# yoseph007/PQA2

Hardware: AMD Instinct MI355X
Metric: VMAF frames/sec (vif+adm+motion2 -> SVM), device-resident synthetic YUV pairs (higher is better)
Workload: dtype f32; 1 GPU; 2160p 3840x2160 8-bit, vmaf_4k_v0.6.1, 300 frames/GPU; frames_per_gpu=300, frames_total=300, batch=97, frames_per_launch=75, clips_pipelined=True, parallelism=frame-shard x1, 1-frame motion halo, all-gather of records + of scores

## Files before the change

### include/pqa_vmaf.h

```cpp
#ifndef PQA_VMAF_H
#define PQA_VMAF_H

#include <stddef.h>
#include <stdint.h>

#if defined(__GNUC__)
#define PQA_API __attribute__((visibility("default")))
#else
#define PQA_API
#endif

#ifdef __cplusplus
extern "C" {
#endif

typedef enum pqa_status {
  PQA_OK = 0,
  PQA_EINVAL = -1,
  PQA_EDEVICE = -2,
  PQA_ENOMEM = -3,
  PQA_ECANCELLED = -4,
  PQA_ESTATE = -5
} pqa_status;

// ... 217 lines not shown
PQA_API int pqa_cross_sse_device(pqa_ctx* ctx, const void* ref_luma, int64_t ref_row_pitch, int64_t ref_frame_pitch,
                                 int32_t n_ref, const void* dis_luma, int64_t dis_row_pitch, int64_t dis_frame_pitch,
                                 int32_t n_dis, int32_t k_lo, int32_t k_hi, uint64_t* out);

PQA_API int pqa_cross_sse(pqa_ctx* ctx, const void* const* ref_frames, int64_t ref_row_stride, int32_t n_ref,
                          const void* const* dis_frames, int64_t dis_row_stride, int32_t n_dis, int32_t k_lo, int32_t k_hi,
                          uint64_t* out);

PQA_API int pqa_shift_sse_device(pqa_ctx* ctx, const void* ref_luma, int64_t ref_row_pitch, int64_t ref_frame_pitch,
                                 const void* dis_luma, int64_t dis_row_pitch, int64_t dis_frame_pitch, int32_t n_frames,
                                 int32_t radius, uint64_t* out);

PQA_API int pqa_shift_sse(pqa_ctx* ctx, const void* const* ref_frames, int64_t ref_row_stride, const void* const* dis_frames,
                          int64_t dis_row_stride, int32_t n_frames, int32_t radius, uint64_t* out);

PQA_API int pqa_level_stats_device(pqa_ctx* ctx, const void* ref, int64_t ref_row_pitch, int64_t ref_frame_pitch,
                                   const void* dis, int64_t dis_row_pitch, int64_t dis_frame_pitch, int32_t n_frames,
                                   int32_t plane, uint64_t* out);

PQA_API int pqa_level_stats(pqa_ctx* ctx, const void* const* ref_frames, int64_t ref_row_stride, const void* const* dis_frames,
                            int64_t dis_row_stride, int32_t n_frames, int32_t plane, uint64_t* out);

PQA_API int pqa_level_bins(const pqa_ctx* ctx);

enum { PQA_RESAMPLE_BILINEAR = 0, PQA_RESAMPLE_BICUBIC = 1, PQA_RESAMPLE_LANCZOS3 = 2 };
typedef struct pqa_resample_spec {
  uint32_t struct_size, filter;
  uint32_t src_width, src_height, dst_width, dst_height;
  int64_t x0_q16, y0_q16, w_q16, h_q16;
} pqa_resample_spec;
PQA_API int pqa_resample(pqa_ctx* ctx, const pqa_resample_spec* spec, const void* const* src_frames, int64_t src_row_stride,
                         void* const* dst_frames, int64_t dst_row_stride, int32_t n_frames);
PQA_API int pqa_resample_device(pqa_ctx* ctx, const pqa_resample_spec* spec, const void* src, int64_t src_row_pitch,
                                int64_t src_frame_pitch, void* dst, int64_t dst_row_pitch, int64_t dst_frame_pitch,
                                int32_t n_frames);

typedef struct pqa_unpack_spec {
  uint32_t struct_size, format;
  uint32_t width, height;
} pqa_unpack_spec;
PQA_API int pqa_unpack_device(pqa_ctx* ctx, const pqa_unpack_spec* spec, const void* src, int64_t src_row_pitch,
                              int64_t src_frame_pitch, int32_t n_frames, const pqa_device_clip* dst);
PQA_API int pqa_unpack(pqa_ctx* ctx, const pqa_unpack_spec* spec, const void* const* src_frames, int64_t src_row_stride,
                       int32_t n_frames, void* const* dst_planes, const int64_t dst_strides[3]);

enum { PQA_SITE_COSITED = 0, PQA_SITE_CENTRE = 1 };
enum { PQA_CONVERT_GENERIC = 1 };
typedef struct pqa_convert_spec {
  uint32_t struct_size, flags;
  uint32_t src_bits, dst_bits;
  uint32_t luma_width, luma_height;
  uint8_t src_hshift, src_vshift, dst_hshift, dst_vshift;
  uint8_t src_hsite, src_vsite, dst_hsite, dst_vsite;
} pqa_convert_spec;
PQA_API int pqa_format_convert(pqa_ctx* ctx, const pqa_convert_spec* spec, const void* const* src_frames, int64_t src_row_stride,
                               void* const* dst_frames, int64_t dst_row_stride, int32_t n_frames);
PQA_API int pqa_format_convert_device(pqa_ctx* ctx, const pqa_convert_spec* spec, const void* src, int64_t src_row_pitch,
                                      int64_t src_frame_pitch, void* dst, int64_t dst_row_pitch, int64_t dst_frame_pitch,
                                      int32_t n_frames);

typedef struct pqa_flow_spec {
  uint32_t struct_size;
  uint32_t width, height;
  uint32_t tile;
} pqa_flow_spec;
PQA_API int pqa_flow_moments(pqa_ctx* ctx, const pqa_flow_spec* spec, const void* const* ref_frames, int64_t ref_row_stride,
                             const void* const* dis_frames, int64_t dis_row_stride, int32_t n_frames, int64_t* out);
PQA_API int pqa_flow_moments_device(pqa_ctx* ctx, const pqa_flow_spec* spec, const void* ref, int64_t ref_row_pitch,
                                    int64_t ref_frame_pitch, const void* dis, int64_t dis_row_pitch, int64_t dis_frame_pitch,
                                    int32_t n_frames, int64_t* out);

typedef struct pqa_profile_spec {
  uint32_t struct_size;
  uint32_t width, height;
} pqa_profile_spec;
PQA_API int pqa_line_profiles(pqa_ctx* ctx, const pqa_profile_spec* spec, const void* const* frames, int64_t row_stride,
                              int32_t n_frames, uint64_t* out);
PQA_API int pqa_line_profiles_device(pqa_ctx* ctx, const pqa_profile_spec* spec, const void* planes, int64_t row_pitch,
                                     int64_t frame_pitch, int32_t n_frames, uint64_t* out);

typedef struct pqa_tile_spec {
  uint32_t struct_size;
  uint32_t width, height;
  uint32_t tile;
} pqa_tile_spec;
PQA_API int pqa_tile_moments(pqa_ctx* ctx, const pqa_tile_spec* spec, const void* const* ref_frames, int64_t ref_row_stride,
                             const void* const* dis_frames, int64_t dis_row_stride, int32_t n_frames, uint64_t* out);
PQA_API int pqa_tile_moments_device(pqa_ctx* ctx, const pqa_tile_spec* spec, const void* ref, int64_t ref_row_pitch,
                                    int64_t ref_frame_pitch, const void* dis, int64_t dis_row_pitch, int64_t dis_frame_pitch,
                                    int32_t n_frames, uint64_t* out);

typedef struct pqa_band_spec {
  uint32_t struct_size;
  uint32_t width, height;
  uint32_t levels;
} pqa_band_spec;
PQA_API int pqa_band_moments(pqa_ctx* ctx, const pqa_band_spec* spec, const void* const* ref_frames, int64_t ref_row_stride,
                             const void* const* dis_frames, int64_t dis_row_stride, int32_t n_frames, uint64_t* out);
PQA_API int pqa_band_moments_device(pqa_ctx* ctx, const pqa_band_spec* spec, const void* ref, int64_t ref_row_pitch,
                                    int64_t ref_frame_pitch, const void* dis, int64_t dis_row_pitch, int64_t dis_frame_pitch,
                                    int32_t n_frames, uint64_t* out);
PQA_API int pqa_band_sums(void);

typedef struct pqa_temporal_spec {
  uint32_t struct_size;
  uint32_t width, height;
  uint32_t tile;
} pqa_temporal_spec;
PQA_API int pqa_temporal_moments(pqa_ctx* ctx, const pqa_temporal_spec* spec, const void* const* ref_frames,
                                 int64_t ref_row_stride, const void* const* dis_frames, int64_t dis_row_stride, int32_t n_frames,
                                 uint64_t* out);
PQA_API int pqa_temporal_moments_device(pqa_ctx* ctx, const pqa_temporal_spec* spec, const void* ref, int64_t ref_row_pitch,
                                        int64_t ref_frame_pitch, const void* dis, int64_t dis_row_pitch, int64_t dis_frame_pitch,
                                        int32_t n_frames, uint64_t* out);
PQA_API int pqa_temporal_sums(void);

typedef struct pqa_edge_spec {
  uint32_t struct_size;
  uint32_t width, height;
} pqa_edge_spec;
PQA_API int pqa_edge_profiles(pqa_ctx* ctx, const pqa_edge_spec* spec, const void* const* ref_frames, int64_t ref_row_stride,
                              const void* const* dis_frames, int64_t dis_row_stride, int32_t n_frames, uint64_t* out);
PQA_API int pqa_edge_profiles_device(pqa_ctx* ctx, const pqa_edge_spec* spec, const void* ref, int64_t ref_row_pitch,
                                     int64_t ref_frame_pitch, const void* dis, int64_t dis_row_pitch, int64_t dis_frame_pitch,
                                     int32_t n_frames, uint64_t* out);
PQA_API int pqa_edge_sums(void);

PQA_API int pqa_colour_sums(void);
PQA_API int pqa_colour_moments_device(pqa_ctx* ctx, const pqa_device_clip* ref, const pqa_device_clip* dis, int32_t n_frames,
                                      uint32_t lo, uint32_t hi, uint64_t* out);
PQA_API int pqa_colour_moments(pqa_ctx* ctx, const void* const* ref_frames, const int64_t ref_strides[3],
                               const void* const* dis_frames, const int64_t dis_strides[3], int32_t n_frames, uint32_t lo,
                               uint32_t hi, uint64_t* out);

PQA_API int pqa_colour_apply_device(pqa_ctx* ctx, const int32_t m[12], const pqa_device_clip* src, const pqa_device_clip* dst,
                                    int32_t n_frames);
PQA_API int pqa_colour_apply(pqa_ctx* ctx, const int32_t m[12], const void* const* src_frames, const int64_t src_strides[3],
                             void* const* dst_frames, const int64_t dst_strides[3], int32_t n_frames);

enum { PQA_GRAY_LUMA = 0, PQA_GRAY_BT601_FULL = 1 };
PQA_API int pqa_set_luma_gray(pqa_ctx* ctx, uint32_t mode);

enum { PQA_PROF_KERNELS = 17 };
PQA_API int pqa_profile_enable(pqa_ctx* ctx, int on);
PQA_API int pqa_profile_read(pqa_ctx* ctx, int kernel_id, double* total_ms, uint64_t* launches, uint64_t* frames);
PQA_API const char* pqa_profile_kernel_name(int kernel_id);

PQA_API int pqa_debug_vif_march_table(uint16_t* out, int32_t capacity_halfwords);

PQA_API int pqa_debug_vif_march_shape(uint32_t width, uint32_t height, int32_t* out6);

PQA_API int pqa_debug_vif_strip_shape(pqa_ctx* ctx, uint32_t scale, uint32_t n_frames, int32_t* out4);

PQA_API int pqa_debug_ciede2000(const double* lab_pairs, int32_t n, double* de_out);

enum { PQA_CAMBI_PARAM_INTS = 22 };
PQA_API int pqa_debug_cambi_params(uint32_t w, uint32_t h, uint32_t bit_depth, int32_t* out, int32_t cap);

PQA_API int pqa_debug_cambi_cmap(const void* luma, int64_t row_pitch_bytes, uint32_t w, uint32_t h, uint32_t bit_depth,
                                 float* cmap, int64_t cap, double* score);

PQA_API int pqa_debug_psnr_hvs_dct8x8(const int32_t* in, int32_t* out, int32_t n);

enum { PQA_PSNR_HVS_TABLE_FLOATS = 384 };
PQA_API int pqa_debug_psnr_hvs_tables(float* out, int32_t cap);

PQA_API int pqa_debug_psnr_hvs_plane(const void* ref, const void* dis, int64_t row_pitch_bytes, uint32_t w, uint32_t h,
                                     uint32_t bit_depth, uint32_t plane_kind, float* block_err, double* mse);

PQA_API int pqa_debug_xpsnr_blocks(const void* ref, const void* ref_m1, const void* ref_m2, const void* dis,
                                   int64_t row_pitch_bytes, uint32_t w, uint32_t h, uint32_t bit_depth, int32_t hfr,
                                   uint64_t* out, double* wsse);

PQA_API int pqa_debug_siti_plane(const void* cur, const void* prev, int64_t row_pitch_bytes, uint32_t w, uint32_t h,
                                 uint32_t bit_depth, int32_t full_range, float* gmap, double* si_ti);

PQA_API int pqa_debug_resample_table(uint32_t filter, int32_t n_src, int32_t n_dst, int64_t x0_q16, int64_t ext_q16,
                                     int32_t* first, int16_t* coeff, int32_t cap_taps, int32_t* taps);

PQA_API int pqa_debug_colour(uint32_t bit_depth, uint32_t hshift, uint32_t vshift, uint32_t w, uint32_t h,
                             const void* const ref[3], const void* const dis[3], uint32_t lo, uint32_t hi, uint64_t* sums28,
                             const int32_t* m, void* const applied[3]);

#ifdef __cplusplus
}
#endif
#endif
```

### pqa2_amd/_native.py

```python
from __future__ import annotations

import ctypes as C
import os
import subprocess

_HERE = os.path.dirname(os.path.abspath(__file__))
LIB_PATH = os.environ.get("PQA_LIB_PATH") or os.path.join(_HERE, "csrc", "libpqa_vmaf.so")

PQA_OK, PQA_EINVAL, PQA_EDEVICE, PQA_ENOMEM, PQA_ECANCELLED, PQA_ESTATE = 0, -1, -2, -3, -4, -5
FEAT_VIF, FEAT_ADM, FEAT_MOTION, FEAT_PSNR, FEAT_SSIM = 1, 2, 4, 8, 16
FEAT_VMAF = FEAT_VIF | FEAT_ADM | FEAT_MOTION
FEAT_ALL = FEAT_VMAF | FEAT_PSNR | FEAT_SSIM
FEAT_FLOAT_SSIM, FEAT_MS_SSIM = 32, 64
FEAT_CIEDE = 256
FEAT_CAMBI, FEAT_CAMBI_FULL_REF = 512, 1024
FEAT_PSNR_HVS = 2048
FEAT_XPSNR, FEAT_XPSNR_HFR = 4096, 8192
FEAT_SITI, FEAT_SITI_REF_FULL, FEAT_SITI_DIS_FULL = 16384, 32768, 65536
FEAT_INTEGRITY = 131072
FEAT_KNOWN = (FEAT_ALL | FEAT_FLOAT_SSIM | FEAT_MS_SSIM | FEAT_CIEDE | FEAT_CAMBI | FEAT_CAMBI_FULL_REF | FEAT_PSNR_HVS
              | FEAT_XPSNR | FEAT_XPSNR_HFR | FEAT_SITI | FEAT_SITI_REF_FULL | FEAT_SITI_DIS_FULL
              | FEAT_INTEGRITY)
VIF_BORDER_FLOAT, VIF_BORDER_INTEGER = 0, 1
FIXED_VIF, FIXED_MOTION, FIXED_ADM, FIXED_ALL = 1, 2, 4, 7
REC_VIF_NUM, REC_VIF_DEN, REC_ADM_NUM, REC_ADM_DEN, REC_MOTION, REC_SSIM, REC_SSE = 0, 4, 8, 12, 16, 17, 20
RECORD_DOUBLES = 24
EXT_FLOAT_SSIM, EXT_FLOAT_SSIM_LCS, EXT_MS_SSIM, EXT_MS_SSIM_L, EXT_MS_SSIM_C, EXT_MS_SSIM_S, EXT_RESERVED = 0, 1, 4, 5, 10, 15, 20
EXT_CIEDE2000, EXT_CIEDE_MEAN_DE = 20, 21
EXT_CAMBI, EXT_CAMBI_SOURCE = 22, 23
CAMBI_PARAM_INTS = 22
EXT_DOUBLES = 24
EXT2_PSNR_HVS_Y, EXT2_PSNR_HVS_CB, EXT2_PSNR_HVS_CR, EXT2_PSNR_HVS, EXT2_PSNR_HVS_MSE, EXT2_RESERVED = 0, 1, 2, 3, 4, 7
EXT2_DOUBLES = 8
EXT3_XPSNR_Y, EXT3_XPSNR_U, EXT3_XPSNR_V, EXT3_WSSE, EXT3_RESERVED = 0, 1, 2, 3, 6
EXT3_DOUBLES = 8
EXT4_SI, EXT4_TI, EXT4_SI_SOURCE, EXT4_TI_SOURCE, EXT4_RESERVED = 0, 1, 2, 3, 4
EXT4_DOUBLES = 8
EXT5_SAD_PREV, EXT5_BLACK_COUNT, EXT5_RESERVED = 0, 3, 4
EXT5_DOUBLES = 8
EXT_BLOCKS = (
    ("ext", EXT_DOUBLES, FEAT_FLOAT_SSIM | FEAT_MS_SSIM | FEAT_CIEDE | FEAT_CAMBI),
    ("ext2", EXT2_DOUBLES, FEAT_PSNR_HVS),
    ("ext3", EXT3_DOUBLES, FEAT_XPSNR),
    ("ext4", EXT4_DOUBLES, FEAT_SITI),
    ("ext5", EXT5_DOUBLES, FEAT_INTEGRITY),
)
PSNR_HVS_TABLE_FLOATS = 384
PROF_KERNELS = 17
GRAY_LUMA, GRAY_BT601_FULL = 0, 1

EXPORTS = [
    "pqa_version", "pqa_record_doubles", "pqa_ext_doubles", "pqa_ext2_doubles", "pqa_ext3_doubles", "pqa_ext4_doubles", "pqa_ext5_doubles", "pqa_config_init", "pqa_create", "pqa_destroy", "pqa_set_stream",
    "pqa_submit", "pqa_submit_fd", "pqa_submit_fd_run", "pqa_submit_device", "pqa_submit_surfaces", "pqa_submit_packed", "pqa_set_motion_halo", "pqa_set_ref_history", "pqa_set_dis_history", "pqa_set_dis_history_planes", "pqa_set_black_threshold", "pqa_frame_sad", "pqa_frame_sad_device", "pqa_flush", "pqa_collect", "pqa_collect_ext", "pqa_collect_ext2", "pqa_collect_ext3", "pqa_collect_ext4", "pqa_collect_ext5", "pqa_sync",
    "pqa_cancel", "pqa_reset", "pqa_last_error", "pqa_luma_stats_device", "pqa_luma_stats", "pqa_cross_sse_device", "pqa_cross_sse", "pqa_shift_sse_device", "pqa_shift_sse", "pqa_level_stats_device", "pqa_level_stats", "pqa_level_bins", "pqa_resample", "pqa_resample_device", "pqa_unpack", "pqa_unpack_device", "pqa_format_convert", "pqa_format_convert_device", "pqa_flow_moments", "pqa_flow_moments_device", "pqa_line_profiles", "pqa_line_profiles_device", "pqa_tile_moments", "pqa_tile_moments_device", "pqa_band_moments", "pqa_band_moments_device", "pqa_band_sums", "pqa_temporal_moments", "pqa_temporal_moments_device", "pqa_temporal_sums", "pqa_edge_profiles", "pqa_edge_profiles_device", "pqa_edge_sums", "pqa_colour_sums", "pqa_colour_moments", "pqa_colour_moments_device", "pqa_colour_apply", "pqa_colour_apply_device", "pqa_set_luma_gray",
    "pqa_profile_enable",
    "pqa_profile_read", "pqa_profile_kernel_name", "pqa_debug_vif_march_table", "pqa_debug_vif_march_shape", "pqa_debug_vif_strip_shape",
    "pqa_debug_ciede2000", "pqa_debug_cambi_params", "pqa_debug_cambi_cmap", "pqa_debug_psnr_hvs_dct8x8",
    "pqa_debug_psnr_hvs_tables", "pqa_debug_psnr_hvs_plane", "pqa_debug_xpsnr_blocks", "pqa_debug_siti_plane",
    "pqa_debug_resample_table", "pqa_debug_colour",
]


class PqaConfig(C.Structure):
    _fields_ = [
        ("struct_size", C.c_uint32), ("device", C.c_int32), ("width", C.c_uint32), ("height", C.c_uint32),
        ("bit_depth", C.c_uint32), ("n_planes", C.c_uint32), ("chroma_hshift", C.c_uint32),
        ("chroma_vshift", C.c_uint32), ("features", C.c_uint32), ("max_batch", C.c_uint32),
        ("result_capacity", C.c_uint32), ("n_subsample", C.c_uint32),
        ("vif_enhn_gain_limit", C.c_double), ("adm_enhn_gain_limit", C.c_double),
        ("vif_border", C.c_uint32), ("fixed_point", C.c_uint32),
    ]


class PqaDeviceClip(C.Structure):
    _fields_ = [("plane", C.c_void_p * 3), ("row_pitch", C.c_int64 * 3), ("frame_pitch", C.c_int64 * 3)]


SURFACE_NV12, SURFACE_P01X = 1, 2
SURFACE_PLANAR, SURFACE_UYVY, SURFACE_YUYV, SURFACE_V210 = 0, 3, 4, 5
PACKED_FORMATS = {"uyvy422": SURFACE_UYVY, "yuyv422": SURFACE_YUYV, "v210": SURFACE_V210}
PACKED_BIT_DEPTH = {SURFACE_UYVY: 8, SURFACE_YUYV: 8, SURFACE_V210: 10}


class PqaSurfaceClip(C.Structure):
    _fields_ = [("struct_size", C.c_uint32), ("format", C.c_uint32), ("luma", C.c_void_p), ("chroma", C.c_void_p),
                ("luma_row_pitch", C.c_int64), ("luma_frame_pitch", C.c_int64),
                ("chroma_row_pitch", C.c_int64), ("chroma_frame_pitch", C.c_int64)]


class PqaHostClip(C.Structure):
    _fields_ = [("struct_size", C.c_uint32), ("format", C.c_uint32), ("frames", C.POINTER(C.c_void_p)), ("strides", C.c_int64 * 3)]


class PqaUnpackSpec(C.Structure):
    _fields_ = [("struct_size", C.c_uint32), ("format", C.c_uint32), ("width", C.c_uint32), ("height", C.c_uint32)]


SITE_COSITED, SITE_CENTRE = 0, 1
CONVERT_GENERIC = 1
CONVERT_BIT_DEPTHS = (8, 10, 12)


class PqaConvertSpec(C.Structure):
    _fields_ = [("struct_size", C.c_uint32), ("flags", C.c_uint32), ("src_bits", C.c_uint32), ("dst_bits", C.c_uint32),
                ("luma_width", C.c_uint32), ("luma_height", C.c_uint32),
                ("src_hshift", C.c_uint8), ("src_vshift", C.c_uint8), ("dst_hshift", C.c_uint8), ("dst_vshift", C.c_uint8),
                ("src_hsite", C.c_uint8), ("src_vsite", C.c_uint8), ("dst_hsite", C.c_uint8), ("dst_vsite", C.c_uint8)]


RESAMPLE_BILINEAR, RESAMPLE_BICUBIC, RESAMPLE_LANCZOS3 = 0, 1, 2
RESAMPLE_FILTERS = {"bilinear": RESAMPLE_BILINEAR, "bicubic": RESAMPLE_BICUBIC, "lanczos": RESAMPLE_LANCZOS3}
RESAMPLE_MAX_TAPS = 32


class PqaResampleSpec(C.Structure):
    _fields_ = [("struct_size", C.c_uint32), ("filter", C.c_uint32), ("src_width", C.c_uint32), ("src_height", C.c_uint32),
                ("dst_width", C.c_uint32), ("dst_height", C.c_uint32), ("x0_q16", C.c_int64), ("y0_q16", C.c_int64),
                ("w_q16", C.c_int64), ("h_q16", C.c_int64)]


FLOW_TILES = (8, 16, 32, 64)
COLOUR_SUMS = 28
COLOUR_Q = 14
COLOUR_MAX_GAIN, COLOUR_MAX_OFFSET = 1 << 16, 1 << 28


class PqaFlowSpec(C.Structure):
    _fields_ = [("struct_size", C.c_uint32), ("width", C.c_uint32), ("height", C.c_uint32), ("tile", C.c_uint32)]


class PqaProfileSpec(C.Structure):
    _fields_ = [("struct_size", C.c_uint32), ("width", C.c_uint32), ("height", C.c_uint32)]


PROFILE_STRIPE, PROFILE_BAND = 1024, 64


class PqaTileSpec(C.Structure):
    _fields_ = [("struct_size", C.c_uint32), ("width", C.c_uint32), ("height", C.c_uint32), ("tile", C.c_uint32)]


TILE_SUMS, TILE_CHUNK = 6, 8


class PqaBandSpec(C.Structure):
    _fields_ = [("struct_size", C.c_uint32), ("width", C.c_uint32), ("height", C.c_uint32), ("levels", C.c_uint32)]


BAND_SUMS, BAND_CHUNK = 3, 8


class PqaTemporalSpec(C.Structure):
    _fields_ = [("struct_size", C.c_uint32), ("width", C.c_uint32), ("height", C.c_uint32), ("tile", C.c_uint32)]


TEMPORAL_SUMS, TEMPORAL_CHUNK = 7, 8
TEMPORAL_SIGNED = (0, 1, 4, 5)


class PqaEdgeSpec(C.Structure):
    _fields_ = [("struct_size", C.c_uint32), ("width", C.c_uint32), ("height", C.c_uint32)]


EDGE_STRIPE, EDGE_BAND = 1024, 64
EDGE_SUMS, EDGE_CHUNK = 3, 8


class PqaError(RuntimeError):
    def __init__(self, code: int, msg: str):
        super().__init__(f"pqa error {code}: {msg}")
        self.code = code


class PqaCancelled(PqaError):
    pass


def build(force: bool = False) -> str:
    script = os.path.join(_HERE, "csrc", "build.sh")
    if force:
        for f in os.listdir(os.path.join(_HERE, "csrc")):
            if f.endswith(".o"):
                os.remove(os.path.join(_HERE, "csrc", f))
    r = subprocess.run(["bash", script], capture_output=True, text=True)
    if r.returncode != 0:
        raise RuntimeError(f"hipcc build failed:\n{r.stdout}\n{r.stderr}")
    return LIB_PATH


_lib = None


def load():
    global _lib
    if _lib is not None:
        return _lib
    if not os.path.exists(LIB_PATH):
        raise ImportError(
            f"{LIB_PATH} is missing: the MI355X HIP extension is not built (run `python -c 'import "
            f"__graft_entry__ as g; g.build()'` or pqa2_amd/csrc/build.sh).  There is no CPU fallback.")
    try:
        import torch
    except Exception:
        pass
    lib = C.CDLL(LIB_PATH)
    missing = [s for s in EXPORTS if not hasattr(lib, s)]
    if missing:
        raise ImportError(f"{LIB_PATH} lacks symbols {missing}")
    vp, i32, i64, dbl = C.c_void_p, C.c_int32, C.c_int64, C.c_double
    lib.pqa_version.restype = C.c_char_p
    lib.pqa_record_doubles.restype = C.c_int
    lib.pqa_config_init.argtypes = [C.POINTER(PqaConfig), C.c_uint32, C.c_uint32]
    lib.pqa_config_init.restype = None
    lib.pqa_create.argtypes = [C.POINTER(PqaConfig), C.POINTER(vp)]
    lib.pqa_destroy.argtypes = [vp]
    lib.pqa_destroy.restype = None
    lib.pqa_set_stream.argtypes = [vp, vp]
    lib.pqa_submit.argtypes = [vp, i64, C.POINTER(vp * 3), C.POINTER(i64 * 3), C.POINTER(vp * 3), C.POINTER(i64 * 3)]
    lib.pqa_submit_fd.argtypes = [vp, i64, C.c_int, C.POINTER(i64 * 3), C.c_int, C.POINTER(i64 * 3)]
    lib.pqa_submit_fd_run.argtypes = [vp, i64, i32, C.c_int, C.POINTER(i64 * 3), i64, C.c_int, C.POINTER(i64 * 3), i64]
    lib.pqa_submit_device.argtypes = [vp, i64, i32, C.POINTER(PqaDeviceClip), C.POINTER(PqaDeviceClip), vp, i64]
    lib.pqa_submit_surfaces.argtypes = [vp, i64, i32, C.POINTER(PqaSurfaceClip), C.POINTER(PqaSurfaceClip),
                                        C.POINTER(PqaSurfaceClip)]
    lib.pqa_submit_packed.argtypes = [vp, i64, i32, C.POINTER(PqaHostClip), C.POINTER(PqaHostClip)]
    lib.pqa_set_motion_halo.argtypes = [vp, vp, i64]
    lib.pqa_flush.argtypes = [vp]
    lib.pqa_collect.argtypes = [vp, i64, i32, vp]
    lib.pqa_collect_ext.argtypes = [vp, i64, i32, vp, vp]
    lib.pqa_ext_doubles.restype = C.c_int
    lib.pqa_collect_ext2.argtypes = [vp, i64, i32, vp, vp, vp]
    lib.pqa_ext2_doubles.restype = C.c_int
    lib.pqa_collect_ext3.argtypes = [vp, i64, i32, vp, vp, vp, vp]
    lib.pqa_ext3_doubles.restype = C.c_int
    lib.pqa_set_ref_history.argtypes = [vp, vp, i32, i64]
    lib.pqa_collect_ext4.argtypes = [vp, i64, i32, vp, vp, vp, vp, vp]
    lib.pqa_ext4_doubles.restype = C.c_int
    lib.pqa_set_dis_history.argtypes = [vp, vp, i64]
    lib.pqa_collect_ext5.argtypes = [vp, i64, i32, vp, vp, vp, vp, vp, vp]
    lib.pqa_ext5_doubles.restype = C.c_int
    lib.pqa_set_dis_history_planes.argtypes = [vp, C.POINTER(vp * 3), C.POINTER(i64 * 3)]
    lib.pqa_set_black_threshold.argtypes = [vp, C.c_uint32]
    lib.pqa_frame_sad.argtypes = [vp, C.POINTER(vp * 3), C.POINTER(i64 * 3), C.POINTER(vp), C.POINTER(i64 * 3), i32, vp]
    lib.pqa_frame_sad_device.argtypes = [vp, C.POINTER(vp * 3), C.POINTER(i64 * 3), C.POINTER(PqaDeviceClip), i32, vp]
    lib.pqa_sync.argtypes = [vp]
    lib.pqa_cancel.argtypes = [vp]
    lib.pqa_luma_stats_device.argtypes = [vp, vp, i64, i64, i32, C.c_uint32, vp]
    lib.pqa_luma_stats.argtypes = [vp, C.POINTER(vp), i64, i32, C.c_uint32, vp]
    lib.pqa_cross_sse_device.argtypes = [vp, vp, i64, i64, i32, vp, i64, i64, i32, i32, i32, vp]
    lib.pqa_cross_sse.argtypes = [vp, C.POINTER(vp), i64, i32, C.POINTER(vp), i64, i32, i32, i32, vp]
    lib.pqa_shift_sse_device.argtypes = [vp, vp, i64, i64, vp, i64, i64, i32, i32, vp]
    lib.pqa_shift_sse.argtypes = [vp, C.POINTER(vp), i64, C.POINTER(vp), i64, i32, i32, vp]
    lib.pqa_level_stats_device.argtypes = [vp, vp, i64, i64, vp, i64, i64, i32, i32, vp]
    lib.pqa_level_stats.argtypes = [vp, C.POINTER(vp), i64, C.POINTER(vp), i64, i32, i32, vp]
    lib.pqa_level_bins.argtypes = [vp]
    lib.pqa_resample.argtypes = [vp, C.POINTER(PqaResampleSpec), C.POINTER(vp), i64, C.POINTER(vp), i64, i32]
    lib.pqa_resample_device.argtypes = [vp, C.POINTER(PqaResampleSpec), vp, i64, i64, vp, i64, i64, i32]
    lib.pqa_unpack_device.argtypes = [vp, C.POINTER(PqaUnpackSpec), vp, i64, i64, i32, C.POINTER(PqaDeviceClip)]
    lib.pqa_format_convert.argtypes = [vp, C.POINTER(PqaConvertSpec), C.POINTER(vp), i64, C.POINTER(vp), i64, i32]
    lib.pqa_format_convert_device.argtypes = [vp, C.POINTER(PqaConvertSpec), vp, i64, i64, vp, i64, i64, i32]
    lib.pqa_unpack.argtypes = [vp, C.POINTER(PqaUnpackSpec), C.POINTER(vp), i64, i32, C.POINTER(vp), C.POINTER(i64 * 3)]
    lib.pqa_flow_moments.argtypes = [vp, C.POINTER(PqaFlowSpec), C.POINTER(vp), i64, C.POINTER(vp), i64, i32, vp]
    lib.pqa_flow_moments_device.argtypes = [vp, C.POINTER(PqaFlowSpec), vp, i64, i64, vp, i64, i64, i32, vp]
    lib.pqa_line_profiles.argtypes = [vp, C.POINTER(PqaProfileSpec), C.POINTER(vp), i64, i32, vp]
    lib.pqa_line_profiles_device.argtypes = [vp, C.POINTER(PqaProfileSpec), vp, i64, i64, i32, vp]
    lib.pqa_tile_moments.argtypes = [vp, C.POINTER(PqaTileSpec), C.POINTER(vp), i64, C.POINTER(vp), i64, i32, vp]
    lib.pqa_tile_moments_device.argtypes = [vp, C.POINTER(PqaTileSpec), vp, i64, i64, vp, i64, i64, i32, vp]
    lib.pqa_band_moments.argtypes = [vp, C.POINTER(PqaBandSpec), C.POINTER(vp), i64, C.POINTER(vp), i64, i32, vp]
    lib.pqa_band_moments_device.argtypes = [vp, C.POINTER(PqaBandSpec), vp, i64, i64, vp, i64, i64, i32, vp]
    lib.pqa_temporal_moments.argtypes = [vp, C.POINTER(PqaTemporalSpec), C.POINTER(vp), i64, C.POINTER(vp), i64, i32, vp]
    lib.pqa_temporal_moments_device.argtypes = [vp, C.POINTER(PqaTemporalSpec), vp, i64, i64, vp, i64, i64, i32, vp]
    lib.pqa_temporal_sums.argtypes = []
    lib.pqa_temporal_sums.restype = C.c_int
    lib.pqa_edge_profiles.argtypes = [vp, C.POINTER(PqaEdgeSpec), C.POINTER(vp), i64, C.POINTER(vp), i64, i32, vp]
    lib.pqa_edge_profiles_device.argtypes = [vp, C.POINTER(PqaEdgeSpec), vp, i64, i64, vp, i64, i64, i32, vp]
    lib.pqa_edge_sums.argtypes = []
    lib.pqa_edge_sums.restype = C.c_int
    lib.pqa_band_sums.argtypes = []
    lib.pqa_band_sums.restype = C.c_int
    lib.pqa_colour_sums.argtypes = []
    lib.pqa_colour_sums.restype = C.c_int
    lib.pqa_colour_moments_device.argtypes = [vp, C.POINTER(PqaDeviceClip), C.POINTER(PqaDeviceClip), i32, C.c_uint32, C.c_uint32, vp]
    lib.pqa_colour_moments.argtypes = [vp, C.POINTER(vp), C.POINTER(i64 * 3), C.POINTER(vp), C.POINTER(i64 * 3), i32, C.c_uint32, C.c_uint32, vp]
    lib.pqa_colour_apply_device.argtypes = [vp, C.POINTER(i32 * 12), C.POINTER(PqaDeviceClip), C.POINTER(PqaDeviceClip), i32]
    lib.pqa_colour_apply.argtypes = [vp, C.POINTER(i32 * 12), C.POINTER(vp), C.POINTER(i64 * 3), C.POINTER(vp), C.POINTER(i64 * 3), i32]
    lib.pqa_debug_colour.argtypes = [C.c_uint32, C.c_uint32, C.c_uint32, C.c_uint32, C.c_uint32, C.POINTER(vp * 3), C.POINTER(vp * 3),
                                     C.c_uint32, C.c_uint32, vp, C.POINTER(i32 * 12), C.POINTER(vp * 3)]
    lib.pqa_debug_resample_table.argtypes = [C.c_uint32, i32, i32, i64, i64, vp, vp, i32, C.POINTER(i32)]
    lib.pqa_set_luma_gray.argtypes = [vp, C.c_uint32]
    lib.pqa_reset.argtypes = [vp]
    lib.pqa_last_error.argtypes = [vp]
    lib.pqa_last_error.restype = C.c_char_p
    lib.pqa_profile_enable.argtypes = [vp, C.c_int]
    lib.pqa_profile_read.argtypes = [vp, C.c_int, C.POINTER(dbl), C.POINTER(C.c_uint64), C.POINTER(C.c_uint64)]
    lib.pqa_debug_vif_march_table.argtypes = [vp, i32]
    lib.pqa_debug_vif_march_shape.argtypes = [C.c_uint32, C.c_uint32, C.POINTER(i32 * 6)]
    lib.pqa_debug_vif_strip_shape.argtypes = [vp, C.c_uint32, C.c_uint32, C.POINTER(i32 * 4)]
    lib.pqa_debug_ciede2000.argtypes = [vp, i32, vp]
    lib.pqa_debug_cambi_params.argtypes = [C.c_uint32, C.c_uint32, C.c_uint32, vp, i32]
    lib.pqa_debug_cambi_cmap.argtypes = [vp, C.c_int64, C.c_uint32, C.c_uint32, C.c_uint32, vp, C.c_int64, vp]
    lib.pqa_debug_psnr_hvs_dct8x8.argtypes = [vp, vp, i32]
    lib.pqa_debug_psnr_hvs_tables.argtypes = [vp, i32]
    lib.pqa_debug_psnr_hvs_plane.argtypes = [vp, vp, C.c_int64, C.c_uint32, C.c_uint32, C.c_uint32, C.c_uint32, vp, vp]
    lib.pqa_debug_xpsnr_blocks.argtypes = [vp, vp, vp, vp, C.c_int64, C.c_uint32, C.c_uint32, C.c_uint32, i32, vp, vp]
    lib.pqa_debug_siti_plane.argtypes = [vp, vp, C.c_int64, C.c_uint32, C.c_uint32, C.c_uint32, i32, vp, vp]
    lib.pqa_profile_kernel_name.argtypes = [C.c_int]
    lib.pqa_profile_kernel_name.restype = C.c_char_p
    assert lib.pqa_record_doubles() == RECORD_DOUBLES
    assert lib.pqa_ext_doubles() == EXT_DOUBLES
    assert lib.pqa_ext2_doubles() == EXT2_DOUBLES
    assert lib.pqa_ext3_doubles() == EXT3_DOUBLES
    assert lib.pqa_ext4_doubles() == EXT4_DOUBLES
    assert lib.pqa_ext5_doubles() == EXT5_DOUBLES
    assert lib.pqa_colour_sums() == COLOUR_SUMS
    _lib = lib
    return lib
```

### pqa2_amd/csrc/adm.hip

```cpp
#include "kernels.h"
#include "pqa_device.h"

namespace pqa {
namespace {

struct AdmArgs {
  const void* ref;
  const void* dis;
  int64_t row_pitch_r, frame_pitch_r, row_pitch_d, frame_pitch_d;
  int w, h, ow, oh, tiles_x, n_tiles;
  float inv_scale, gain_limit, rf_hv, rf_d;
  float k_hv, k_d;
  int left, top, right, bottom;
  float* ll_ref;
  float* ll_dis;
  int64_t ll_row_pitch_r, ll_frame_pitch_r, ll_row_pitch_d, ll_frame_pitch_d;
  double* partials;
};

constexpr int TW = kAdmTileW, TH = kAdmTileH, GW = TW + 2, GH = TH + 2, NRP = GH / 2;
constexpr int VC = 2 * GW + 2, VP = 128;
static_assert(VC <= 128 && VC <= VP && GH % 2 == 0 && GW <= 64, "one column per lane, rows in pairs");
constexpr int SROWS = GH / 2;
constexpr int NIN = 2 * SROWS + 2;
// ... 98 lines not shown
    const int lcyA = 2 * rp, cyA = cy0 - 1 + lcyA, cyB = cyA + 1;
    f2 s[4][4];
#pragma unroll
    for (int q = 0; q < 4; ++q) {
      if (LLONLY && (q & 1)) continue;
      const f4* p = reinterpret_cast<const f4*>(&V[q][rp][2 * lcxs]);
      const f4 v01 = p[0], v23 = p[1];
      s[q][0] = f2{v01.x, v01.y}; s[q][1] = f2{v01.z, v01.w};
      s[q][2] = f2{v23.x, v23.y}; s[q][3] = f2{v23.z, v23.w};
    }
#define PQA_DWT(c0, c1, c2, c3, t)                                                                        \
  __builtin_elementwise_fma(splat(c3), t[3],                                                              \
                            __builtin_elementwise_fma(splat(c2), t[2], __builtin_elementwise_fma(splat(c1), t[1], splat(c0) * t[0])))
    const f2 ra = PQA_DWT(lo0, lo1, lo2, lo3, s[0]);
    const f2 da = PQA_DWT(lo0, lo1, lo2, lo3, s[2]);
    const bool vA = col_valid && cyA >= 0 && cyA < a.oh, vB = col_valid && cyB >= 0 && cyB < a.oh;
    const bool iA = col_inner && lcyA >= 1 && cyA < a.oh;
    const bool iB = col_inner && lcyA + 1 <= TH && cyB >= 0 && cyB < a.oh;
    if (a.ll_ref) {
      float* lr = a.ll_ref + (int64_t)fr * a.ll_frame_pitch_r;
      float* ld = a.ll_dis + (int64_t)fr * a.ll_frame_pitch_d;
      if (iA) {
        lr[(unsigned)cyA * (unsigned)a.ll_row_pitch_r + (unsigned)cx] = ra.x;
        ld[(unsigned)cyA * (unsigned)a.ll_row_pitch_d + (unsigned)cx] = da.x;
      }
      if (iB) {
        lr[(unsigned)cyB * (unsigned)a.ll_row_pitch_r + (unsigned)cx] = ra.y;
        ld[(unsigned)cyB * (unsigned)a.ll_row_pitch_d + (unsigned)cx] = da.y;
      }
    }
    if (LLONLY) continue;
    const f2 ov = PQA_DWT(hi0, hi1, hi2, hi3, s[0]);
    const f2 oh = PQA_DWT(lo0, lo1, lo2, lo3, s[1]);
    const f2 od = PQA_DWT(hi0, hi1, hi2, hi3, s[1]);
    const f2 tv = PQA_DWT(hi0, hi1, hi2, hi3, s[2]);
    const f2 th = PQA_DWT(lo0, lo1, lo2, lo3, s[3]);
    const f2 td = PQA_DWT(hi0, hi1, hi2, hi3, s[3]);
#undef PQA_DWT
    const f2 ot_dp = __builtin_elementwise_fma(ov, tv, oh * th);
    const f2 o_mag_sq = __builtin_elementwise_fma(ov, ov, oh * oh), t_mag_sq = __builtin_elementwise_fma(tv, tv, th * th);
    const f2 lhs = ot_dp * ot_dp, rhs = splat(cos_1deg_sq) * o_mag_sq * t_mag_sq;
    const bool angA = (ot_dp.x >= 0.0f) && (lhs.x >= rhs.x), angB = (ot_dp.y >= 0.0f) && (lhs.y >= rhs.y);
    const f2 z2 = splat(0.0f);
    const f2 m2 = f2{angA ? a.gain_limit : 1.0f, angB ? a.gain_limit : 1.0f};
    const f2 rh = med3_2(z2, th, oh * m2), rv = med3_2(z2, tv, ov * m2), rd = med3_2(z2, td, od * m2);
    const f2 ah = th - rh, av = tv - rv, ad = td - rd;
    const float gA = fmaf(a.k_d, fabsf(ad.x), a.k_hv * (fabsf(ah.x) + fabsf(av.x)));
    const float gB = fmaf(a.k_d, fabsf(ad.y), a.k_hv * (fabsf(ah.y) + fabsf(av.y)));
    const bool wA = iA && col_win && cyA >= a.top && cyA < a.bottom;
    const bool wB = iB && col_win && cyB >= a.top && cyB < a.bottom;
    const f2 mw = f2{wA ? 1.0f : 0.0f, wB ? 1.0f : 0.0f};
    mwin[k] = mw;
    xs[k][0] = rh * splat(a.rf_hv);
    xs[k][1] = rv * splat(a.rf_hv);
    xs[k][2] = rd * splat(a.rf_d);
    const f2 qh = mw * (oh * oh), qv = mw * (ov * ov), qd = mw * (od * od);
    den_h = f2{fmaf(qh.x, fabsf(oh.x), den_h.x), fmaf(qh.y, fabsf(oh.y), den_h.y)};
    den_v = f2{fmaf(qv.x, fabsf(ov.x), den_v.x), fmaf(qv.y, fabsf(ov.y), den_v.y)};
    den_d = f2{fmaf(qd.x, fabsf(od.x), den_d.x), fmaf(qd.y, fabsf(od.y), den_d.y)};
    if (have) {
      G[lcyA][lcx] = vA ? gA : 0.0f;
      G[lcyA + 1][lcx] = vB ? gB : 0.0f;
    }
  }
  if (LLONLY) {
    if (tid < 6) a.partials[((int64_t)fr * a.n_tiles + tile) * 6 + tid] = 0.0;
    return;
  }
  __syncthreads();

  f2 num_h = f2{0.0f, 0.0f}, num_v = num_h, num_d = num_h;
  {
    const int lx0 = min(max(mirror1(cx - 1, a.ow) - (cx0 - 1), 0), GW - 1);
    const int lx2 = min(max(mirror1(cx + 1, a.ow) - (cx0 - 1), 0), GW - 1);
#pragma unroll
    for (int k = 0; k < NROUND; ++k) {
      const int rp = wave + 4 * k;
      const int lcyA = 2 * rp, cyA = cy0 - 1 + lcyA;
      int ly[4] = {mirror1(cyA - 1, a.oh) - (cy0 - 1), lcyA, lcyA + 1, mirror1(cyA + 2, a.oh) - (cy0 - 1)};
      ly[0] = min(max(ly[0], 0), GH - 1);
      ly[3] = min(max(ly[3], 0), GH - 1);
      float rs[4], c[2];
#pragma unroll
      for (int j = 0; j < 4; ++j) {
        const float m = G[ly[j]][lcxs];
        rs[j] = G[ly[j]][lx0] + m + G[ly[j]][lx2];
        if (j == 1) c[0] = m;
        if (j == 2) c[1] = m;
      }
      const float downA = (cyA + 1 < a.oh) ? rs[2] : rs[1];
      const float upB = (cyA >= 0) ? rs[1] : rs[3];
      const f2 thr = f2{(rs[0] + rs[1] + downA) + c[0], (upB + rs[2] + rs[3]) + c[1]};
      const f2 mw = mwin[k];
#pragma unroll
      for (int t = 0; t < 3; ++t) {
        f2 x = f2{fmaxf(fabsf(xs[k][t].x) - thr.x, 0.0f), fmaxf(fabsf(xs[k][t].y) - thr.y, 0.0f)};
        const f2 x3 = (mw * x) * (x * x);
        if (t == 0) num_h += x3;
        if (t == 1) num_v += x3;
        if (t == 2) num_d += x3;
      }
    }
  }
  const float rf3_hv = a.rf_hv * a.rf_hv * a.rf_hv, rf3_d = a.rf_d * a.rf_d * a.rf_d;
  const float part[6] = {num_h.x + num_h.y, num_v.x + num_v.y, num_d.x + num_d.y,
                         rf3_hv * (den_h.x + den_h.y), rf3_hv * (den_v.x + den_v.y), rf3_d * (den_d.x + den_d.y)};
  double v[6];
  block_sum_f32<6>(part, v, red);
  if (tid == 0) {
    double* out = a.partials + ((int64_t)fr * a.n_tiles + tile) * 6;
#pragma unroll
    for (int i = 0; i < 6; ++i) out[i] = v[i];
  }
}

template <typename T>
__global__ __launch_bounds__(kBlock, 4) void adm_scale_kernel(const AdmArgs a) {
  __shared__ f2 V[4][NRP][VP];
  __shared__ float G[GH][GP];
  __shared__ double red[24];
  const int tile = xcd_remap(blockIdx.x, a.n_tiles);
  const int tx = tile % a.tiles_x, ty = tile / a.tiles_x;
  const int fr = blockIdx.y;
  const int cx0 = tx * TW, cy0 = ty * TH;
  const bool outside = !(cx0 < a.right && cx0 + TW > a.left && cy0 < a.bottom && cy0 + TH > a.top);
  if (outside) {
    if (!a.ll_ref) {
      if (threadIdx.x < 6) a.partials[((int64_t)fr * a.n_tiles + tile) * 6 + threadIdx.x] = 0.0;
      return;
    }
    adm_tile<T, true>(a, V, G, red, tile, tx, ty, fr);
  } else {
    adm_tile<T, false>(a, V, G, red, tile, tx, ty, fr);
  }
}

static float dwt_quant_step(int lambda, int theta) {
  static const double g[3] = {1.501, 1.0, 0.534};
  static const double amp[4][3] = {{0.62171, 0.67234, 0.72709},
                                   {0.34537, 0.41317, 0.49428},
                                   {0.18004, 0.22727, 0.28688},
                                   {0.091401, 0.11792, 0.15214}};
  const float r = (float)(3.0 * 1080 * M_PI / 180.0);
  const float temp = (float)log10(pow(2.0, lambda + 1) * 0.401 * g[theta] / (double)r);
  return (float)(2.0 * 0.495 * pow(10.0, 0.466 * (double)temp * (double)temp) / amp[lambda][theta]);
}

}

float adm_dwt_quant_step(int lambda, int theta) { return dwt_quant_step(lambda, theta); }

hipError_t launch_adm_scale(hipStream_t stream, int scale, Elem elem, PlaneRun ref, PlaneRun dis, int n_frames,
                            int w, int h, float inv_scale, float gain_limit, MutPlaneRun ll_ref,
                            MutPlaneRun ll_dis, double* partials, int mode, int* n_partials) {
  if (n_partials) *n_partials = adm_tiles_x((w + 1) / 2) * adm_tiles_y((h + 1) / 2);
  if (n_frames <= 0) return hipSuccess;
  if (mode != ADM_TILED) {
    hipError_t err = hipSuccess;
    if (launch_adm_march(stream, scale, elem, ref, dis, n_frames, w, h, inv_scale, gain_limit, ll_ref, ll_dis, partials,
                         n_partials, &err))
      return err;
  }
  AdmArgs a{};
  a.ref = ref.base; a.dis = dis.base;
  a.row_pitch_r = ref.row_pitch; a.frame_pitch_r = ref.frame_pitch;
  a.row_pitch_d = dis.row_pitch; a.frame_pitch_d = dis.frame_pitch;
  a.w = w; a.h = h;
  a.ow = (w + 1) / 2; a.oh = (h + 1) / 2;
  a.tiles_x = adm_tiles_x(a.ow);
  a.n_tiles = a.tiles_x * adm_tiles_y(a.oh);
  a.inv_scale = inv_scale; a.gain_limit = gain_limit;
  a.rf_hv = 1.0f / dwt_quant_step(scale, 1);
  a.rf_d = 1.0f / dwt_quant_step(scale, 2);
  a.k_hv = a.rf_hv / 30.0f;
  a.k_d = a.rf_d / 30.0f;
  const double border = 0.1;
  a.left = (int)(a.ow * border - 0.5);
  a.top = (int)(a.oh * border - 0.5);
  a.right = a.ow - a.left;
  a.bottom = a.oh - a.top;
  a.ll_ref = (float*)ll_ref.base; a.ll_dis = (float*)ll_dis.base;
  a.ll_row_pitch_r = ll_ref.row_pitch; a.ll_frame_pitch_r = ll_ref.frame_pitch;
  a.ll_row_pitch_d = ll_dis.row_pitch; a.ll_frame_pitch_d = ll_dis.frame_pitch;
  a.partials = partials;
  const dim3 grid(a.n_tiles, n_frames), block(kBlock);
  switch (elem) {
    case ELEM_U8: hipLaunchKernelGGL((adm_scale_kernel<uint8_t>), grid, block, 0, stream, a); break;
    case ELEM_U16: hipLaunchKernelGGL((adm_scale_kernel<uint16_t>), grid, block, 0, stream, a); break;
    case ELEM_F32: hipLaunchKernelGGL((adm_scale_kernel<float>), grid, block, 0, stream, a); break;
  }
  return hipGetLastError();
}

}
```

### pqa2_amd/csrc/adm_march.hip

```cpp
#include <type_traits>

#include "adm_chain.h"
#include "kernels.h"
#include "pqa_device.h"

namespace pqa {
namespace {

constexpr int kStripe = 60;
constexpr int kHalo = 2;

struct AdmMarchArgs {
  const void* ref;
  const void* dis;
  unsigned pitch_r, pitch_d;
  int64_t frame_pitch_r, frame_pitch_d;
  int w, h, ow, oh;
  int aligned;
  int n_stripes, n_sg;
  int n_frames;
  int left, top, right, bottom;
  int reg_start[4];
  int seg_rows[3], seg_first[4];
  float inv_scale, gain_limit, rf_hv, rf_d, k_hv, k_d;
  float* ll_ref;
  float* ll_dis;
  unsigned ll_pitch_r, ll_pitch_d;
  int64_t ll_frame_pitch_r, ll_frame_pitch_d;
  double* partials;
  int n_part;
};

using namespace admc;

template <typename T, bool EDGE> struct RawRow;
template <> struct RawRow<uint8_t, false> { unsigned r, d; };
template <> struct RawRow<uint16_t, false> { unsigned r, d; };
template <> struct RawRow<float, false> { f2 r, d; };
template <typename T> struct RawRow<T, true> { T r0, r1, d0, d1; };
template <> struct RawRow<float, true> { f2 c0, c1; };

template <typename T, bool EDGE>
struct RowLoader {
  rsrc_t rsrc_r, rsrc_d;
  unsigned v0, v1;
  unsigned pitch_r, pitch_d;
  int h;
  float inv_scale;

  __device__ __forceinline__ RawRow<T, EDGE> load(int y ) const {
    const unsigned gy = (unsigned)mirror1(y, h);
    const unsigned so_r = gy * pitch_r, so_d = gy * pitch_d;
    RawRow<T, EDGE> o;
    if constexpr (EDGE && sizeof(T) == 4) {
      o.c0 = f2{buf_load<T>(rsrc_r, v0, so_r), buf_load<T>(rsrc_d, v0, so_d)};
      o.c1 = f2{buf_load<T>(rsrc_r, v1, so_r), buf_load<T>(rsrc_d, v1, so_d)};
    } else if constexpr (EDGE) {
      o.r0 = buf_load<T>(rsrc_r, v0, so_r); o.r1 = buf_load<T>(rsrc_r, v1, so_r);
      o.d0 = buf_load<T>(rsrc_d, v0, so_d); o.d1 = buf_load<T>(rsrc_d, v1, so_d);
    } else if constexpr (sizeof(T) == 1) {
      o.r = (unsigned short)__builtin_amdgcn_raw_buffer_load_b16(rsrc_r, v0, so_r, 0);
      o.d = (unsigned short)__builtin_amdgcn_raw_buffer_load_b16(rsrc_d, v0, so_d, 0);
    } else if constexpr (sizeof(T) == 2) {
      o.r = __builtin_amdgcn_raw_buffer_load_b32(rsrc_r, v0 * 2u, so_r * 2u, 0);
      o.d = __builtin_amdgcn_raw_buffer_load_b32(rsrc_d, v0 * 2u, so_d * 2u, 0);
    } else {
      o.r = __builtin_bit_cast(f2, __builtin_amdgcn_raw_buffer_load_b64(rsrc_r, v0 * 4u, so_r * 4u, 0));
      o.d = __builtin_bit_cast(f2, __builtin_amdgcn_raw_buffer_load_b64(rsrc_d, v0 * 4u, so_d * 4u, 0));
    }
    return o;
  }
  __device__ __forceinline__ Row convert(const RawRow<T, EDGE>& x) const {
    if constexpr (EDGE && sizeof(T) == 4) {
      return Row{x.c0, x.c1};
    } else if constexpr (EDGE) {
      return Row{PixIO<T>::pair(x.r0, x.d0, inv_scale), PixIO<T>::pair(x.r1, x.d1, inv_scale)};
    } else if constexpr (sizeof(T) == 1) {
      return Row{PixIO<T>::pair((uint8_t)(x.r & 0xffu), (uint8_t)(x.d & 0xffu), inv_scale),
                 PixIO<T>::pair((uint8_t)((x.r >> 8) & 0xffu), (uint8_t)((x.d >> 8) & 0xffu), inv_scale)};
    } else if constexpr (sizeof(T) == 2) {
      return Row{PixIO<T>::pair((uint16_t)(x.r & 0xffffu), (uint16_t)(x.d & 0xffffu), inv_scale),
                 PixIO<T>::pair((uint16_t)(x.r >> 16), (uint16_t)(x.d >> 16), inv_scale)};
    } else {
      return Row{f2{x.r.x, x.d.x}, f2{x.r.y, x.d.y}};
    }
  }
};

template <typename T, bool EDGE>
__device__ __forceinline__ void march_full(const AdmMarchArgs& a, const RowLoader<T, EDGE>& ld, const int lane, const int cs,
                                           const int r0, const int r1, float* __restrict__ ll_r, float* __restrict__ ll_d,
                                           const unsigned ll_voff, double* __restrict__ part) {
  const Consts K{a.gain_limit, a.rf_hv, a.rf_d, a.k_hv, a.k_d};
  const rsrc_t ll_rs_r = make_rsrc(ll_r, ll_r ? (unsigned)a.oh * a.ll_pitch_r * 4u : 0u);
  const rsrc_t ll_rs_d = make_rsrc(ll_d, ll_d ? (unsigned)a.oh * a.ll_pitch_d * 4u : 0u);
  const bool fix_left = EDGE && cs == 0;
  const int lane_m1 = mirror1(-1, a.ow) + kHalo;
  const int lane_ow = a.ow - (cs - kHalo);
  const bool fix_right = EDGE && lane_ow <= 63;

  float acc[6] = {0.0f, 0.0f, 0.0f, 0.0f, 0.0f, 0.0f};
  double dacc[6] = {0.0, 0.0, 0.0, 0.0, 0.0, 0.0};

  const auto row = [&](const Row& xa, const Row& xb, const Row& xc, const Row& xd, const int i, auto own, Pending& p) -> float {
    constexpr bool OWN = decltype(own)::value;
    const f2 vl0 = dwt_lo(xa.c0, xb.c0, xc.c0, xd.c0), vl1 = dwt_lo(xa.c1, xb.c1, xc.c1, xd.c1);
    const f2 vh0 = dwt_hi(xa.c0, xb.c0, xc.c0, xd.c0), vh1 = dwt_hi(xa.c1, xb.c1, xc.c1, xd.c1);
    const f2 vlm = from_left(vl1), vlp = from_right(vl0), vhm = from_left(vh1), vhp = from_right(vh0);
    const f2 bv = dwt_hi(vlm, vl0, vl1, vlp);
    const f2 bh = dwt_lo(vhm, vh0, vh1, vhp);
    const f2 bd = dwt_hi(vhm, vh0, vh1, vhp);
    if (OWN) {
      const f2 ba = dwt_lo(vlm, vl0, vl1, vlp);
      store_f32(ba.x, ll_rs_r, ll_voff, (unsigned)i * a.ll_pitch_r * 4u);
      store_f32(ba.y, ll_rs_d, ll_voff, (unsigned)i * a.ll_pitch_d * 4u);
    }
    float g = decouple(bh, bv, bd, K, p);
    if (EDGE) {
      if (fix_left) {
        const float g1 = __builtin_bit_cast(float, __builtin_amdgcn_readlane(__builtin_bit_cast(int, g), lane_m1));
        g = lane == kHalo - 1 ? g1 : g;
      }
      if (fix_right) {
        const float gl = __builtin_bit_cast(float, __builtin_amdgcn_readlane(__builtin_bit_cast(int, g), lane_ow - 1));
        g = lane == lane_ow ? gl : g;
      }
    }
    p.g = g;
    if (OWN) den_accumulate(bh, bv, bd, acc + 3);
    return (from_left(g) + g) + from_right(g);
  };
  const auto finish_row = [&](const Pending& p, const float s2, const float rs_below) { finish(p, s2, rs_below, K, acc); };
  const auto flush = [&]() {
#pragma unroll
    for (int q = 0; q < 6; ++q) { dacc[q] += (double)acc[q]; acc[q] = 0.0f; }
  };
  const std::integral_constant<bool, true> own{};
  const std::integral_constant<bool, false> guest{};

  Row w0, w1, w2, w3;
  float rs_prev, s2 = 0.0f;
  Pending pa{0.0f, 0.0f, 0.0f, 0.0f}, pb = pa;
  {
    const int wi = mirror1(r0 - 1, a.oh);
    w0 = ld.convert(ld.load(2 * wi - 1)); w1 = ld.convert(ld.load(2 * wi));
    w2 = ld.convert(ld.load(2 * wi + 1)); w3 = ld.convert(ld.load(2 * wi + 2));
    Pending unused;
    rs_prev = row(w0, w1, w2, w3, wi, guest, unused);
    if (wi != r0 - 1) {
      w2 = ld.convert(ld.load(2 * r0 - 1)); w3 = ld.convert(ld.load(2 * r0));
    }
  }
  RawRow<T, EDGE> qa0 = ld.load(2 * r0 + 1), qa1 = ld.load(2 * r0 + 2), qb0 = ld.load(2 * r0 + 3), qb1 = ld.load(2 * r0 + 4);
  const auto step = [&](const Row& c0, const Row& c1, Row& n0, Row& n1, const Pending& above, Pending& mine,
                        RawRow<T, EDGE>& q0, RawRow<T, EDGE>& q1, const int i, auto is_own) {
    n0 = ld.convert(q0); n1 = ld.convert(q1);
    if (decltype(is_own)::value) { q0 = ld.load(2 * i + 5); q1 = ld.load(2 * i + 6); }
    const float rs = row(c0, c1, n0, n1, i, is_own, mine);
    finish_row(above, s2, rs);
    s2 = rs_prev + rs;
    rs_prev = rs;
  };
  int i = r0;
  for (; i + 1 < r1; i += 2) {
    step(w2, w3, w0, w1, pa, pb, qa0, qa1, i, own);
    step(w0, w1, w2, w3, pb, pa, qb0, qb1, i + 1, own);
    if (((i - r0) & 6) == 6) flush();
  }
  if (i < r1) {
    step(w2, w3, w0, w1, pa, pb, qa0, qa1, i, own);
    w2 = w0; w3 = w1; pa = pb; qa0 = qb0; qa1 = qb1;
  }
  if (r1 < a.oh) {
    step(w2, w3, w0, w1, pa, pb, qa0, qa1, r1, guest);
  } else {
    finish_row(pa, s2, rs_prev);
  }
  flush();
  const int c = cs - kHalo + lane;
  const bool col_win = lane >= kHalo && lane < kHalo + kStripe && c >= a.left && c < a.right;
  const double rf3_hv = (double)(a.rf_hv * a.rf_hv * a.rf_hv), rf3_d = (double)(a.rf_d * a.rf_d * a.rf_d);
#pragma unroll
  for (int q = 0; q < 6; ++q) {
    double v = wave_sum(col_win ? dacc[q] : 0.0);
    if (q >= 3) v *= q == 5 ? rf3_d : rf3_hv;
    if (lane == 0) part[q] = v;
  }
}

template <typename T, bool EDGE>
__device__ __forceinline__ void march_ll(const AdmMarchArgs& a, const RowLoader<T, EDGE>& ld, const int r0, const int r1,
                                         float* __restrict__ ll_r, float* __restrict__ ll_d, const unsigned ll_voff) {
  const rsrc_t ll_rs_r = make_rsrc(ll_r, (unsigned)a.oh * a.ll_pitch_r * 4u);
  const rsrc_t ll_rs_d = make_rsrc(ll_d, (unsigned)a.oh * a.ll_pitch_d * 4u);
  Row w0, w1, w2, w3;
  w2 = ld.convert(ld.load(2 * r0 - 1)); w3 = ld.convert(ld.load(2 * r0));
  RawRow<T, EDGE> qa0 = ld.load(2 * r0 + 1), qa1 = ld.load(2 * r0 + 2), qb0 = ld.load(2 * r0 + 3), qb1 = ld.load(2 * r0 + 4);
  const auto step = [&](const Row& c0, const Row& c1, Row& n0, Row& n1, RawRow<T, EDGE>& q0, RawRow<T, EDGE>& q1, const int i) {
    n0 = ld.convert(q0); n1 = ld.convert(q1);
    q0 = ld.load(2 * i + 5); q1 = ld.load(2 * i + 6);
    const f2 vl0 = dwt_lo(c0.c0, c1.c0, n0.c0, n1.c0), vl1 = dwt_lo(c0.c1, c1.c1, n0.c1, n1.c1);
    const f2 ba = dwt_lo(from_left(vl1), vl0, vl1, from_right(vl0));
    store_f32(ba.x, ll_rs_r, ll_voff, (unsigned)i * a.ll_pitch_r * 4u);
    store_f32(ba.y, ll_rs_d, ll_voff, (unsigned)i * a.ll_pitch_d * 4u);
  };
  int i = r0;
  for (; i + 1 < r1; i += 2) {
    step(w2, w3, w0, w1, qa0, qa1, i);
    step(w0, w1, w2, w3, qb0, qb1, i + 1);
  }
  if (i < r1) step(w2, w3, w0, w1, qa0, qa1, i);
}

#ifndef PQA_ADM_MARCH_OCC
#define PQA_ADM_MARCH_OCC 4
#endif
template <typename T>
__global__ __launch_bounds__(kBlock, PQA_ADM_MARCH_OCC) void adm_march_kernel(const AdmMarchArgs a) {
  const int tid = threadIdx.x, lane = tid & 63;
  const int wave = __builtin_amdgcn_readfirstlane(tid >> 6);
  const int n_seg = a.seg_first[3];
  const int sg = blockIdx.x % a.n_sg;
  const int t = blockIdx.x / a.n_sg;
  const int fr = t % a.n_frames, k = t / a.n_frames;
  const int seg = (k + a.seg_first[1]) % n_seg;
  const int id = seg * a.n_sg + sg;
  const int stripe = sg * 4 + wave;
  double* __restrict__ part = a.partials + ((int64_t)fr * a.n_part + (int64_t)id * 4 + wave) * 6;
  const int region = seg >= a.seg_first[2] ? 2 : seg >= a.seg_first[1] ? 1 : 0;
  const int r0 = a.reg_start[region] + (seg - a.seg_first[region]) * a.seg_rows[region];
  const int r1 = min(r0 + a.seg_rows[region], a.reg_start[region + 1]);
  const int cs = stripe * kStripe;
  const bool in_win = region == 1 && cs < a.right && cs + kStripe > a.left;
  if (stripe >= a.n_stripes || (!in_win && !a.ll_ref)) {
    if (lane < 6) part[lane] = 0.0;
    return;
  }
  const T* __restrict__ ref = (const T*)a.ref + (int64_t)fr * a.frame_pitch_r;
  const T* __restrict__ dis = (const T*)a.dis + (int64_t)fr * a.frame_pitch_d;
  float* __restrict__ ll_r = a.ll_ref ? a.ll_ref + (int64_t)fr * a.ll_frame_pitch_r : nullptr;
  float* __restrict__ ll_d = a.ll_ref ? a.ll_dis + (int64_t)fr * a.ll_frame_pitch_d : nullptr;
  const int c = cs - kHalo + lane;
  const unsigned ll_voff = (lane >= kHalo && lane < kHalo + kStripe && c < a.ow) ? (unsigned)c * 4u : 0x80000000u;
  const bool fast = a.aligned && cs >= kHalo && 2 * (cs + kStripe + kHalo - 1) + 1 < a.w;
  const unsigned bytes_r = (unsigned)a.h * a.pitch_r * (unsigned)sizeof(T), bytes_d = (unsigned)a.h * a.pitch_d * (unsigned)sizeof(T);
  if (fast) {
    const RowLoader<T, false> ld{make_rsrc(ref, bytes_r), make_rsrc(dis, bytes_d), (unsigned)(2 * c), 0u, a.pitch_r, a.pitch_d, a.h, a.inv_scale};
    if (in_win) {
      march_full<T, false>(a, ld, lane, cs, r0, r1, ll_r, ll_d, ll_voff, part);
    } else {
      march_ll<T, false>(a, ld, r0, r1, ll_r, ll_d, ll_voff);
      if (lane < 6) part[lane] = 0.0;
    }
  } else {
    const RowLoader<T, true> ld{make_rsrc(ref, bytes_r), make_rsrc(dis, bytes_d), (unsigned)mirror1(2 * c, a.w), (unsigned)mirror1(2 * c + 1, a.w),
                                a.pitch_r, a.pitch_d, a.h, a.inv_scale};
    if (in_win) {
      march_full<T, true>(a, ld, lane, cs, r0, r1, ll_r, ll_d, ll_voff, part);
    } else {
      march_ll<T, true>(a, ld, r0, r1, ll_r, ll_d, ll_voff);
      if (lane < 6) part[lane] = 0.0;
    }
  }
}

#ifndef PQA_ADM_SEG_ROWS
#define PQA_ADM_SEG_ROWS 32
#endif
#ifndef PQA_ADM_SEG_MIN
#define PQA_ADM_SEG_MIN 32
#endif
#ifndef PQA_ADM_WAVES
#define PQA_ADM_WAVES 384
#endif

struct Partition {
  int reg_start[4], seg_rows[3], seg_first[4];
};
Partition partition_rows(int oh, int top, int bottom, int n_stripes) {
  Partition p{};
  p.reg_start[0] = 0; p.reg_start[1] = top; p.reg_start[2] = bottom; p.reg_start[3] = oh;
  int first = 0;
  for (int r = 0; r < 3; ++r) {
    const int len = p.reg_start[r + 1] - p.reg_start[r];
    int rows = (len * n_stripes + PQA_ADM_WAVES - 1) / PQA_ADM_WAVES;
    rows = rows < PQA_ADM_SEG_MIN ? PQA_ADM_SEG_MIN : rows > PQA_ADM_SEG_ROWS ? PQA_ADM_SEG_ROWS : rows;
    const int n = (len + rows - 1) / rows;
    p.seg_rows[r] = n ? (len + n - 1) / n : 1;
    p.seg_first[r] = first;
    first += n ? (len + p.seg_rows[r] - 1) / p.seg_rows[r] : 0;
  }
  p.seg_first[3] = first;
  return p;
}

}

int adm_march_partials(int band_w, int band_h) {
  const int top = (int)(band_h * 0.1 - 0.5);
  const int n_stripes = (band_w + kStripe - 1) / kStripe;
  const Partition p = partition_rows(band_h, top, band_h - top, n_stripes);
  return ((n_stripes + 3) / 4) * 4 * p.seg_first[3];
}

bool launch_adm_march(hipStream_t stream, int scale, Elem elem, PlaneRun ref, PlaneRun dis, int n_frames, int w, int h,
                      float inv_scale, float gain_limit, MutPlaneRun ll_ref, MutPlaneRun ll_dis, double* partials,
                      int* n_partials, hipError_t* err) {
  const int es = elem == ELEM_U8 ? 1 : elem == ELEM_U16 ? 2 : 4;
  if ((int64_t)ref.row_pitch * h * es >= (1ll << 31) || (int64_t)dis.row_pitch * h * es >= (1ll << 31)) return false;
  AdmMarchArgs a{};
  a.ref = ref.base; a.dis = dis.base;
  a.pitch_r = (unsigned)ref.row_pitch; a.pitch_d = (unsigned)dis.row_pitch;
  a.frame_pitch_r = ref.frame_pitch; a.frame_pitch_d = dis.frame_pitch;
  a.w = w; a.h = h;
  a.ow = (w + 1) / 2; a.oh = (h + 1) / 2;
  if (ll_ref.base && ((int64_t)ll_ref.row_pitch * a.oh * 4 >= (1ll << 31) || (int64_t)ll_dis.row_pitch * a.oh * 4 >= (1ll << 31))) return false;
  const uintptr_t two = (uintptr_t)(2 * es - 1);
  a.aligned = (((uintptr_t)ref.base | (uintptr_t)dis.base) & two) == 0 &&
              ((ref.row_pitch | dis.row_pitch | ref.frame_pitch | dis.frame_pitch) & 1) == 0;
  a.n_stripes = (a.ow + kStripe - 1) / kStripe;
  a.n_sg = (a.n_stripes + 3) / 4;
  const double border = 0.1;
  a.left = (int)(a.ow * border - 0.5);
  a.top = (int)(a.oh * border - 0.5);
  a.right = a.ow - a.left;
  a.bottom = a.oh - a.top;
  const Partition p = partition_rows(a.oh, a.top, a.bottom, a.n_stripes);
  for (int r = 0; r < 4; ++r) { a.reg_start[r] = p.reg_start[r]; a.seg_first[r] = p.seg_first[r]; }
  for (int r = 0; r < 3; ++r) a.seg_rows[r] = p.seg_rows[r];
  a.inv_scale = inv_scale; a.gain_limit = gain_limit;
  a.rf_hv = 1.0f / adm_dwt_quant_step(scale, 1);
  a.rf_d = 1.0f / adm_dwt_quant_step(scale, 2);
  a.k_hv = a.rf_hv / 30.0f;
  a.k_d = a.rf_d / 30.0f;
  a.ll_ref = (float*)ll_ref.base; a.ll_dis = (float*)ll_dis.base;
  a.ll_pitch_r = (unsigned)ll_ref.row_pitch; a.ll_pitch_d = (unsigned)ll_dis.row_pitch;
  a.ll_frame_pitch_r = ll_ref.frame_pitch; a.ll_frame_pitch_d = ll_dis.frame_pitch;
  a.partials = partials;
  a.n_part = a.n_sg * 4 * p.seg_first[3];
  if (n_partials) *n_partials = a.n_part;
  a.n_frames = n_frames;
  const dim3 grid((unsigned)a.n_sg * p.seg_first[3] * n_frames), block(kBlock);
  switch (elem) {
    case ELEM_U8: hipLaunchKernelGGL((adm_march_kernel<uint8_t>), grid, block, 0, stream, a); break;
    case ELEM_U16: hipLaunchKernelGGL((adm_march_kernel<uint16_t>), grid, block, 0, stream, a); break;
    case ELEM_F32: hipLaunchKernelGGL((adm_march_kernel<float>), grid, block, 0, stream, a); break;
  }
  *err = hipGetLastError();
  return true;
}

}
```

### pqa2_amd/csrc/adm_pyramid.hip

```cpp
#include <type_traits>

#include "adm_chain.h"
#include "kernels.h"
#include "pqa_device.h"

namespace pqa {
namespace {

using namespace admc;

constexpr int kP1 = 60;
constexpr int kPH = 2;

struct PyramidArgs {
  const void* ref;
  const void* dis;
  unsigned pitch_r, pitch_d;
  int64_t frame_pitch_r, frame_pitch_d;
  int w, h, ow0, oh0, ow1, oh1;
  int aligned;
  int n_stripes, n_sg, seg_rows, n_seg;
  int n_frames;
  int left0, top0, right0, bottom0, left1, top1, right1, bottom1;
  float inv_scale;
  Consts k0, k1;
  float* ll_ref;
  float* ll_dis;
  unsigned ll_pitch_r, ll_pitch_d;
  int64_t ll_frame_pitch_r, ll_frame_pitch_d;
  double* part0;
  double* part1;
  int n_part;
};

struct Row4 {
  f2 c[4];
};
template <typename T, bool EDGE> struct Raw4;
template <> struct Raw4<uint8_t, false> { unsigned r, d; };
template <> struct Raw4<uint16_t, false> { unsigned r0, r1, d0, d1; };
template <typename T> struct Raw4<T, true> { T r[4], d[4]; };

template <typename T, bool EDGE>
struct Loader4 {
  rsrc_t rsrc_r, rsrc_d;
  unsigned v[4];
  unsigned pitch_r, pitch_d;
  int h;
  float inv_scale;
  __device__ __forceinline__ Raw4<T, EDGE> load(int y ) const {
    const unsigned gy = (unsigned)mirror1(y, h);
    const unsigned so_r = gy * pitch_r, so_d = gy * pitch_d;
    Raw4<T, EDGE> o;
    if constexpr (EDGE) {
#pragma unroll
      for (int k = 0; k < 4; ++k) { o.r[k] = buf_load<T>(rsrc_r, v[k], so_r); o.d[k] = buf_load<T>(rsrc_d, v[k], so_d); }
    } else if constexpr (sizeof(T) == 1) {
      o.r = __builtin_amdgcn_raw_buffer_load_b32(rsrc_r, v[0], so_r, 0);
      o.d = __builtin_amdgcn_raw_buffer_load_b32(rsrc_d, v[0], so_d, 0);
    } else {
      typedef unsigned u2 __attribute__((ext_vector_type(2)));
      const u2 r = __builtin_bit_cast(u2, __builtin_amdgcn_raw_buffer_load_b64(rsrc_r, v[0] * 2u, so_r * 2u, 0));
      const u2 d = __builtin_bit_cast(u2, __builtin_amdgcn_raw_buffer_load_b64(rsrc_d, v[0] * 2u, so_d * 2u, 0));
      o.r0 = r[0]; o.r1 = r[1]; o.d0 = d[0]; o.d1 = d[1];
    }
    return o;
  }
  __device__ __forceinline__ Row4 convert(const Raw4<T, EDGE>& x) const {
    Row4 o;
    if constexpr (EDGE) {
#pragma unroll
      for (int k = 0; k < 4; ++k) o.c[k] = PixIO<T>::pair(x.r[k], x.d[k], inv_scale);
    } else if constexpr (sizeof(T) == 1) {
      o.c[0] = PixIO<T>::pair((uint8_t)(x.r & 0xffu), (uint8_t)(x.d & 0xffu), inv_scale);
      o.c[1] = PixIO<T>::pair((uint8_t)((x.r >> 8) & 0xffu), (uint8_t)((x.d >> 8) & 0xffu), inv_scale);
      o.c[2] = PixIO<T>::pair((uint8_t)((x.r >> 16) & 0xffu), (uint8_t)((x.d >> 16) & 0xffu), inv_scale);
      o.c[3] = PixIO<T>::pair((uint8_t)(x.r >> 24), (uint8_t)(x.d >> 24), inv_scale);
    } else {
      o.c[0] = PixIO<T>::pair((uint16_t)(x.r0 & 0xffffu), (uint16_t)(x.d0 & 0xffffu), inv_scale);
      o.c[1] = PixIO<T>::pair((uint16_t)(x.r0 >> 16), (uint16_t)(x.d0 >> 16), inv_scale);
      o.c[2] = PixIO<T>::pair((uint16_t)(x.r1 & 0xffffu), (uint16_t)(x.d1 & 0xffffu), inv_scale);
      o.c[3] = PixIO<T>::pair((uint16_t)(x.r1 >> 16), (uint16_t)(x.d1 >> 16), inv_scale);
    }
    return o;
  }
};

struct BoxState {
  float s2 = 0.0f, rs_prev = 0.0f;
  Pending pend{0.0f, 0.0f, 0.0f, 0.0f};
};

template <typename T, bool EDGE>
__device__ __forceinline__ void pyramid_march(const PyramidArgs& a, const Loader4<T, EDGE>& ld, const int lane, const int stripe,
                                              const int R0, const int R1, const int fr, double* __restrict__ part0,
                                              double* __restrict__ part1, double (*dsum)[kBlock]) {
  const int cs1 = stripe * kP1;
  const int c1 = cs1 - kPH + lane;
  const bool inner = lane >= kPH && lane < kPH + kP1;
  const bool win0 = 2 * cs1 < a.right0 && 2 * (cs1 + kP1) > a.left0;
  const bool win1 = cs1 < a.right1 && cs1 + kP1 > a.left1;
  const bool first = EDGE && stripe == 0;
  const int lane_e = a.ow1 - (cs1 - kPH);
  const bool last = EDGE && lane_e <= 63;
  const bool at_m1 = first && lane == kPH - 1, at_e = last && lane == lane_e;

  float* __restrict__ ll_r = a.ll_ref + (int64_t)fr * a.ll_frame_pitch_r;
  float* __restrict__ ll_d = a.ll_dis + (int64_t)fr * a.ll_frame_pitch_d;
  const rsrc_t ll_rs_r = make_rsrc(ll_r, (unsigned)a.oh1 * a.ll_pitch_r * 4u);
  const rsrc_t ll_rs_d = make_rsrc(ll_d, (unsigned)a.oh1 * a.ll_pitch_d * 4u);
  const unsigned ll_voff = (inner && c1 < a.ow1) ? (unsigned)c1 * 4u : 0x80000000u;

  float accA[6] = {0, 0, 0, 0, 0, 0}, accB[6] = {0, 0, 0, 0, 0, 0}, acc1[6] = {0, 0, 0, 0, 0, 0};
  const int tid = threadIdx.x;
#pragma unroll
  for (int q = 0; q < 12; ++q) dsum[q][tid] = 0.0;
  const float mA = (inner && 2 * c1 >= a.left0 && 2 * c1 < a.right0) ? 1.0f : 0.0f;
  const float mB = (inner && 2 * c1 + 1 >= a.left0 && 2 * c1 + 1 < a.right0) ? 1.0f : 0.0f;
  const auto flush = [&]() {
#pragma unroll
    for (int q = 0; q < 6; ++q) {
      dsum[q][tid] += (double)fmaf(mB, accB[q], mA * accA[q]);
      dsum[6 + q][tid] += (double)acc1[q];
      accA[q] = 0.0f; accB[q] = 0.0f; acc1[q] = 0.0f;
    }
  };

  BoxState bxA, bxB, bx1;
  const auto step0 = [&](const Row4& xa, const Row4& xb, const Row4& xc, const Row4& xd, const int i, const bool chain,
                         const bool acc_this, const bool acc_above) -> Row {
    f2 vl[4];
#pragma unroll
    for (int k = 0; k < 4; ++k) vl[k] = dwt_lo(xa.c[k], xb.c[k], xc.c[k], xd.c[k]);
    const f2 vlm = from_left(vl[3]), vlp = from_right(vl[0]);
    Row ll{dwt_lo(vlm, vl[0], vl[1], vl[2]), dwt_lo(vl[1], vl[2], vl[3], vlp)};
    float rsA = 0.0f, rsB = 0.0f;
    Pending pA{0.0f, 0.0f, 0.0f, 0.0f}, pB = pA;
    if (chain) {
      f2 vh[4];
#pragma unroll
      for (int k = 0; k < 4; ++k) vh[k] = dwt_hi(xa.c[k], xb.c[k], xc.c[k], xd.c[k]);
      const f2 vhm = from_left(vh[3]), vhp = from_right(vh[0]);
      const f2 bvA = dwt_hi(vlm, vl[0], vl[1], vl[2]), bhA = dwt_lo(vhm, vh[0], vh[1], vh[2]), bdA = dwt_hi(vhm, vh[0], vh[1], vh[2]);
      const f2 bvB = dwt_hi(vl[1], vl[2], vl[3], vlp), bhB = dwt_lo(vh[1], vh[2], vh[3], vhp), bdB = dwt_hi(vh[1], vh[2], vh[3], vhp);
      float gA = decouple(bhA, bvA, bdA, a.k0, pA);
      float gB = decouple(bhB, bvB, bdB, a.k0, pB);
      if (EDGE) {
        if (first) { const float t = from_right(gB); gB = at_m1 ? t : gB; }
        if (last) { const float t = from_left(gB); gA = at_e ? t : gA; }
      }
      pA.g = gA; pB.g = gB;
      if (acc_this) { den_accumulate(bhA, bvA, bdA, accA + 3); den_accumulate(bhB, bvB, bdB, accB + 3); }
      rsA = (from_left(gB) + gA) + gB;
      rsB = (gA + gB) + from_right(gA);
    }
    if (acc_above) { finish(bxA.pend, bxA.s2, rsA, a.k0, accA); finish(bxB.pend, bxB.s2, rsB, a.k0, accB); }
    bxA.s2 = bxA.rs_prev + rsA; bxA.rs_prev = rsA; bxA.pend = pA;
    bxB.s2 = bxB.rs_prev + rsB; bxB.rs_prev = rsB; bxB.pend = pB;
    (void)i;
    return ll;
  };
  const auto step1 = [&](const Row& xa, const Row& xb, const Row& xc, const Row& xd, const int j, const bool chain, const bool own,
                         const bool acc_this, const bool acc_above) {
    const f2 vl0 = dwt_lo(xa.c0, xb.c0, xc.c0, xd.c0), vl1 = dwt_lo(xa.c1, xb.c1, xc.c1, xd.c1);
    const f2 vlm = from_left(vl1), vlp = from_right(vl0);
    if (own) {
      const f2 ba = dwt_lo(vlm, vl0, vl1, vlp);
      store_f32(ba.x, ll_rs_r, ll_voff, (unsigned)j * a.ll_pitch_r * 4u);
      store_f32(ba.y, ll_rs_d, ll_voff, (unsigned)j * a.ll_pitch_d * 4u);
    }
    float rs = 0.0f;
    Pending p{0.0f, 0.0f, 0.0f, 0.0f};
    if (chain) {
      const f2 vh0 = dwt_hi(xa.c0, xb.c0, xc.c0, xd.c0), vh1 = dwt_hi(xa.c1, xb.c1, xc.c1, xd.c1);
      const f2 vhm = from_left(vh1), vhp = from_right(vh0);
      const f2 bv = dwt_hi(vlm, vl0, vl1, vlp), bh = dwt_lo(vhm, vh0, vh1, vhp), bd = dwt_hi(vhm, vh0, vh1, vhp);
      float g = decouple(bh, bv, bd, a.k1, p);
      if (EDGE) {
        if (first) { const float t = __builtin_bit_cast(float, __builtin_amdgcn_readlane(__builtin_bit_cast(int, g), kPH + 1)); g = at_m1 ? t : g; }
        if (last) { const float t = from_left(g); g = at_e ? t : g; }
      }
      p.g = g;
      if (acc_this) den_accumulate(bh, bv, bd, acc1 + 3);
      rs = (from_left(g) + g) + from_right(g);
    }
    if (acc_above) finish(bx1.pend, bx1.s2, rs, a.k1, acc1);
    bx1.s2 = bx1.rs_prev + rs; bx1.rs_prev = rs; bx1.pend = p;
  };
  const auto band_edges = [&](Row r) -> Row {
    if (EDGE) {
      if (first) { const f2 t = from_right(r.c1); r.c1 = at_m1 ? t : r.c1; }
      if (last) { const f2 t = from_left(r.c1); r.c0 = at_e ? t : r.c0; }
    }
    return r;
  };

  const int j_first = R0 - 1, j_last = R1 < a.oh1 ? R1 : R1 - 1;
  const int i0 = 2 * j_first - 1;
  Row4 x0, x1, x2, x3;
  x2 = ld.convert(ld.load(2 * i0 - 1)); x3 = ld.convert(ld.load(2 * i0));
  Raw4<T, EDGE> q[4];
  q[0] = ld.load(2 * i0 + 1); q[1] = ld.load(2 * i0 + 2); q[2] = ld.load(2 * i0 + 3); q[3] = ld.load(2 * i0 + 4);
  Row u0, u1, v0, v1;
  {
    x0 = ld.convert(q[0]); x1 = ld.convert(q[1]);
    q[0] = ld.load(2 * i0 + 5); q[1] = ld.load(2 * i0 + 6);
    u0 = band_edges(step0(x2, x3, x0, x1, i0, false, false, false));
    x2 = ld.convert(q[2]); x3 = ld.convert(q[3]);
    q[2] = ld.load(2 * i0 + 7); q[3] = ld.load(2 * i0 + 8);
    u1 = band_edges(step0(x0, x1, x2, x3, i0 + 1, false, false, false));
  }
  const auto need0 = [&](int i) { return win0 && i >= a.top0 - 1 && i <= a.bottom0 && i >= 2 * R0 - 1 && i <= 2 * R1; };
  const auto accum0 = [&](int i) { return win0 && i >= a.top0 && i < a.bottom0 && i >= 2 * R0 && i < 2 * R1; };
  const auto need1 = [&](int j) { return win1 && j >= a.top1 - 1 && j <= a.bottom1; };
  const auto accum1 = [&](int j) { return win1 && j >= a.top1 && j < a.bottom1 && j >= R0 && j < R1; };
  const auto iteration = [&](const int j, Row& w0, Row& w1, Row& w2, Row& w3) {
    const int ia = 2 * j + 1, ib = 2 * j + 2;
    x0 = ld.convert(q[0]); x1 = ld.convert(q[1]);
    q[0] = ld.load(2 * ia + 5); q[1] = ld.load(2 * ia + 6);
    w2 = band_edges(step0(x2, x3, x0, x1, ia, need0(ia), accum0(ia), accum0(ia - 1)));
    x2 = ld.convert(q[2]); x3 = ld.convert(q[3]);
    q[2] = ld.load(2 * ib + 5); q[3] = ld.load(2 * ib + 6);
    w3 = band_edges(step0(x0, x1, x2, x3, ib, need0(ib), accum0(ib), accum0(ib - 1)));
    if (j == 0) w0 = w2;
    if (ib == a.oh0) w3 = w2;
    step1(w0, w1, w2, w3, j, need1(j), j >= R0 && j < R1, accum1(j), accum1(j - 1));
  };
  if constexpr (sizeof(T) == 1) {
    for (int j = j_first; j <= j_last; j += 2) {
      iteration(j, u0, u1, v0, v1);
      if (j + 1 <= j_last) {
        iteration(j + 1, v0, v1, u0, u1);
        if (((j + 1 - j_first) & 3) == 3) flush();
      }
    }
  } else {
    for (int j = j_first; j <= j_last; ++j) {
      iteration(j, u0, u1, v0, v1);
      u0 = v0; u1 = v1;
      if (((j - j_first) & 3) == 3) flush();
    }
  }
  flush();
  const bool col1 = inner && c1 >= a.left1 && c1 < a.right1;
  const double rf0_hv = (double)(a.k0.rf_hv * a.k0.rf_hv * a.k0.rf_hv), rf0_d = (double)(a.k0.rf_d * a.k0.rf_d * a.k0.rf_d);
  const double rf1_hv = (double)(a.k1.rf_hv * a.k1.rf_hv * a.k1.rf_hv), rf1_d = (double)(a.k1.rf_d * a.k1.rf_d * a.k1.rf_d);
#pragma unroll
  for (int q6 = 0; q6 < 6; ++q6) {
    double v0 = wave_sum(dsum[q6][tid]);
    double v1 = wave_sum(col1 ? dsum[6 + q6][tid] : 0.0);
    if (q6 >= 3) { v0 *= q6 == 5 ? rf0_d : rf0_hv; v1 *= q6 == 5 ? rf1_d : rf1_hv; }
    if (lane == 0) { part0[q6] = v0; part1[q6] = v1; }
  }
}

#ifndef PQA_ADM_PYRAMID_OCC
#define PQA_ADM_PYRAMID_OCC 3
#endif
template <typename T>
__global__ __launch_bounds__(kBlock, PQA_ADM_PYRAMID_OCC) void adm_pyramid_kernel(const PyramidArgs a) {
  __shared__ double dsum[12][kBlock];
  const int tid = threadIdx.x, lane = tid & 63;
  const int wave = __builtin_amdgcn_readfirstlane(tid >> 6);
#ifdef PQA_ADM_PYRAMID_PLAIN_ORDER
  const int sg = blockIdx.x % a.n_sg, seg = (blockIdx.x / a.n_sg) % a.n_seg, fr = blockIdx.x / (a.n_sg * a.n_seg);
#else
  const int sg = blockIdx.x % a.n_sg;
  const int t = blockIdx.x / a.n_sg;
  const int fr = t % a.n_frames, k = t / a.n_frames;
  const int seg = (a.n_seg - 1) / 2 + ((k & 1) ? (k + 1) / 2 : -(k / 2));
#endif
  const int id = seg * a.n_sg + sg;
  const int stripe = sg * 4 + wave;
  double* __restrict__ part0 = a.part0 + ((int64_t)fr * a.n_part + (int64_t)id * 4 + wave) * 6;
  double* __restrict__ part1 = a.part1 + ((int64_t)fr * a.n_part + (int64_t)id * 4 + wave) * 6;
  if (stripe >= a.n_stripes) {
    if (lane < 6) { part0[lane] = 0.0; part1[lane] = 0.0; }
    return;
  }
  const int R0 = seg * a.seg_rows, R1 = min(R0 + a.seg_rows, a.oh1);
  const T* __restrict__ ref = (const T*)a.ref + (int64_t)fr * a.frame_pitch_r;
  const T* __restrict__ dis = (const T*)a.dis + (int64_t)fr * a.frame_pitch_d;
  const unsigned bytes_r = (unsigned)a.h * a.pitch_r * (unsigned)sizeof(T), bytes_d = (unsigned)a.h * a.pitch_d * (unsigned)sizeof(T);
  const int cs1 = stripe * kP1, c1 = cs1 - kPH + lane;
  const bool fast = a.aligned && cs1 >= kPH && 4 * (cs1 + kP1 + kPH - 1) + 3 < a.w;
  if (fast) {
    const Loader4<T, false> ld{make_rsrc(ref, bytes_r), make_rsrc(dis, bytes_d), {(unsigned)(4 * c1), 0u, 0u, 0u}, a.pitch_r, a.pitch_d, a.h, a.inv_scale};
    pyramid_march<T, false>(a, ld, lane, stripe, R0, R1, fr, part0, part1, dsum);
  } else {
    const Loader4<T, true> ld{make_rsrc(ref, bytes_r), make_rsrc(dis, bytes_d),
                              {(unsigned)mirror1(4 * c1, a.w), (unsigned)mirror1(4 * c1 + 1, a.w), (unsigned)mirror1(4 * c1 + 2, a.w), (unsigned)mirror1(4 * c1 + 3, a.w)},
                              a.pitch_r, a.pitch_d, a.h, a.inv_scale};
    pyramid_march<T, true>(a, ld, lane, stripe, R0, R1, fr, part0, part1, dsum);
  }
}

#ifndef PQA_ADM_PYRAMID_SEG_ROWS
#define PQA_ADM_PYRAMID_SEG_ROWS 32
#endif

}

bool adm_pyramid_takes(Elem elem, int w, int h) {
  return (elem == ELEM_U8 || elem == ELEM_U16) && w % 4 == 0 && h % 4 == 0 && w >= 128 && h >= 128;
}

int adm_pyramid_partials(int w, int h) {
  const int ow1 = w / 4, oh1 = h / 4;
  const int n_stripes = (ow1 + kP1 - 1) / kP1;
  return ((n_stripes + 3) / 4) * 4 * ((oh1 + PQA_ADM_PYRAMID_SEG_ROWS - 1) / PQA_ADM_PYRAMID_SEG_ROWS);
}

bool launch_adm_pyramid(hipStream_t stream, Elem elem, PlaneRun ref, PlaneRun dis, int n_frames, int w, int h, float inv_scale,
                        float gain_limit, MutPlaneRun ll_ref, MutPlaneRun ll_dis, double* partials0, double* partials1,
                        int* n_partials, hipError_t* err) {
  if (!adm_pyramid_takes(elem, w, h) || !ll_ref.base || !ll_dis.base) return false;
  const int es = elem == ELEM_U8 ? 1 : 2;
  if ((int64_t)ref.row_pitch * h * es >= (1ll << 31) || (int64_t)dis.row_pitch * h * es >= (1ll << 31)) return false;
  PyramidArgs a{};
  a.ref = ref.base; a.dis = dis.base;
  a.pitch_r = (unsigned)ref.row_pitch; a.pitch_d = (unsigned)dis.row_pitch;
  a.frame_pitch_r = ref.frame_pitch; a.frame_pitch_d = dis.frame_pitch;
  a.w = w; a.h = h;
  a.ow0 = w / 2; a.oh0 = h / 2; a.ow1 = w / 4; a.oh1 = h / 4;
  if ((int64_t)ll_ref.row_pitch * a.oh1 * 4 >= (1ll << 31) || (int64_t)ll_dis.row_pitch * a.oh1 * 4 >= (1ll << 31)) return false;
  const uintptr_t four = (uintptr_t)(4 * es - 1);
  a.aligned = (((uintptr_t)ref.base | (uintptr_t)dis.base) & four) == 0 &&
              ((ref.row_pitch | dis.row_pitch | ref.frame_pitch | dis.frame_pitch) & 3) == 0;
  a.n_stripes = (a.ow1 + kP1 - 1) / kP1;
  a.n_sg = (a.n_stripes + 3) / 4;
  a.seg_rows = PQA_ADM_PYRAMID_SEG_ROWS;
  a.n_seg = (a.oh1 + a.seg_rows - 1) / a.seg_rows;
  const double border = 0.1;
  a.left0 = (int)(a.ow0 * border - 0.5); a.top0 = (int)(a.oh0 * border - 0.5);
  a.right0 = a.ow0 - a.left0; a.bottom0 = a.oh0 - a.top0;
  a.left1 = (int)(a.ow1 * border - 0.5); a.top1 = (int)(a.oh1 * border - 0.5);
  a.right1 = a.ow1 - a.left1; a.bottom1 = a.oh1 - a.top1;
  if (a.top0 < 2 || a.top1 < 2) return false;
  a.inv_scale = inv_scale;
  for (int s = 0; s < 2; ++s) {
    Consts& k = s ? a.k1 : a.k0;
    k.gain_limit = gain_limit;
    k.rf_hv = 1.0f / adm_dwt_quant_step(s, 1);
    k.rf_d = 1.0f / adm_dwt_quant_step(s, 2);
    k.k_hv = k.rf_hv / 30.0f;
    k.k_d = k.rf_d / 30.0f;
  }
  a.ll_ref = (float*)ll_ref.base; a.ll_dis = (float*)ll_dis.base;
  a.ll_pitch_r = (unsigned)ll_ref.row_pitch; a.ll_pitch_d = (unsigned)ll_dis.row_pitch;
  a.ll_frame_pitch_r = ll_ref.frame_pitch; a.ll_frame_pitch_d = ll_dis.frame_pitch;
  a.part0 = partials0; a.part1 = partials1;
  a.n_part = a.n_sg * 4 * a.n_seg;
  if (n_partials) *n_partials = a.n_part;
  a.n_frames = n_frames;
  const dim3 grid((unsigned)a.n_sg * a.n_seg * n_frames), block(kBlock);
  if (elem == ELEM_U16) hipLaunchKernelGGL((adm_pyramid_kernel<uint16_t>), grid, block, 0, stream, a);
  else hipLaunchKernelGGL((adm_pyramid_kernel<uint8_t>), grid, block, 0, stream, a);
  *err = hipGetLastError();
  return true;
}

}
```

### pqa2_amd/csrc/kernels.h

```cpp
#pragma once
#include <hip/hip_runtime.h>
#include <stdint.h>

#include <vector>

namespace pqa {

enum Elem : int { ELEM_U8 = 0, ELEM_U16 = 1, ELEM_F32 = 2 };

struct PlaneRun {
  const void* base;
  int64_t row_pitch;
  int64_t frame_pitch;
};

struct MutPlaneRun {
  void* base;
  int64_t row_pitch;
  int64_t frame_pitch;
};

int vif_tile_w(int scale);
constexpr int kVifTileH = 8;
inline int vif_tiles_x(int scale, int w) { return (w + vif_tile_w(scale) - 1) / vif_tile_w(scale); }
inline int vif_tiles_y(int h) { return (h + kVifTileH - 1) / kVifTileH; }

enum : int { VIF_S0_VALU = 0, VIF_S0_AUTO = 1 };
hipError_t launch_vif_stat(hipStream_t stream, int scale, Elem elem, PlaneRun ref, PlaneRun dis, int n_frames,
                           int w, int h, float inv_scale, float gain_limit, int border101, double* partials,
                           MutPlaneRun next_ref, MutPlaneRun next_dis, int s0_mode = VIF_S0_AUTO, int* n_partials = nullptr,
                           int uniform = 1, int strip_seg = 0);
void vif_strip_shape(int scale, int w, int h, int n_frames, int strip_seg, int* out4);
hipError_t vif_march_prepare();
int vif_march_partials_max(int w, int h);
int vif_march_table(uint16_t* out, int capacity_halfwords);
void vif_march_shape(int w, int h, int* out6);
bool launch_vif_s0_march(hipStream_t stream, Elem elem, int bits, PlaneRun ref, PlaneRun dis, int n_frames, int w, int h, float gain_limit,
                         int border101, double* partials, MutPlaneRun next_ref, MutPlaneRun next_dis, int* n_partials,
                         hipError_t* err, int uniform = 1);
constexpr int kVifFxPartials = 8;
void vif_fixed_log2_table(uint16_t* out32768);
hipError_t launch_vif_fixed(hipStream_t stream, int scale, int bit_depth, Elem elem, PlaneRun ref, PlaneRun dis,
                            int n_frames, int w, int h, double gain_limit, const uint16_t* log2_lut,
                            long long* partials, MutPlaneRun next_ref, MutPlaneRun next_dis);

constexpr int kAdmTileW = 60, kAdmTileH = 14;
inline int adm_tiles_x(int band_w) { return (band_w + kAdmTileW - 1) / kAdmTileW; }
inline int adm_tiles_y(int band_h) { return (band_h + kAdmTileH - 1) / kAdmTileH; }

enum : int { ADM_TILED = 0, ADM_AUTO = 1, ADM_MARCH = 2 };
hipError_t launch_adm_scale(hipStream_t stream, int scale, Elem elem, PlaneRun ref, PlaneRun dis, int n_frames,
                            int w, int h, float inv_scale, float gain_limit, MutPlaneRun ll_ref,
                            MutPlaneRun ll_dis, double* partials, int mode = ADM_AUTO, int* n_partials = nullptr);
int adm_march_partials(int band_w, int band_h);
bool launch_adm_march(hipStream_t stream, int scale, Elem elem, PlaneRun ref, PlaneRun dis, int n_frames, int w, int h,
                      float inv_scale, float gain_limit, MutPlaneRun ll_ref, MutPlaneRun ll_dis, double* partials,
                      int* n_partials, hipError_t* err);
bool adm_pyramid_takes(Elem elem, int w, int h);
int adm_pyramid_partials(int w, int h);
bool launch_adm_pyramid(hipStream_t stream, Elem elem, PlaneRun ref, PlaneRun dis, int n_frames, int w, int h, float inv_scale,
                        float gain_limit, MutPlaneRun ll_ref, MutPlaneRun ll_dis, double* partials0, double* partials1,
                        int* n_partials, hipError_t* err);
float adm_dwt_quant_step(int lambda, int theta);

constexpr int kAdmFxRows = kAdmTileH + 2;
struct AdmFxScale {
  int scale, band_w, band_h;
  int left, top, right, bottom;
  float rf[3];
  uint32_t i_rf[3];
  int cm_shift_sq[3], cm_shift_sub[3], cm_shift_cub[3], cm_final_q[3];
  int den_shift_sq, den_shift_cub, den_final_q;
  int num_row_shift, den_row_shift;
};
AdmFxScale adm_fixed_scale_params(int scale, int band_w, int band_h);
void adm_fixed_div_table(int32_t* out65537);
void adm_fixed_epilogue(const AdmFxScale& p, const long long acc[6], double* num_out, double* den_out);
hipError_t launch_adm_fixed(hipStream_t stream, int scale, int bit_depth, Elem elem, PlaneRun ref, PlaneRun dis,
                            int n_frames, int w, int h, double gain_limit, const int32_t* div_lut,
                            MutPlaneRun ll_ref, MutPlaneRun ll_dis, long long* partials);

constexpr int kMotionTileW = 252, kMotionTileH = 16;
inline int motion_tiles(int w, int h) {
  return ((w + kMotionTileW - 1) / kMotionTileW) * ((h + kMotionTileH - 1) / kMotionTileH);
}
enum : int { MOTION_TILED = 0, MOTION_AUTO = 1 };
hipError_t launch_motion(hipStream_t stream, Elem elem, PlaneRun ref, const void* prev0, int64_t prev0_row_pitch,
                         int n_frames, int w, int h, float inv_scale, double* partials, int mode = MOTION_AUTO,
                         int* n_partials = nullptr);
int motion_march_partials(int w, int h);
bool launch_motion_march(hipStream_t stream, Elem elem, PlaneRun ref, const void* prev0, int64_t prev0_row_pitch, int n_frames,
                         int w, int h, double* partials, int* n_partials, hipError_t* err);
hipError_t launch_motion_fixed(hipStream_t stream, int bit_depth, Elem elem, PlaneRun ref, const void* prev0,
                               int64_t prev0_row_pitch, int n_frames, int w, int h, unsigned long long* partials);

constexpr int kSseBlocksPerPlane = 256;
hipError_t launch_sse(hipStream_t stream, Elem elem, PlaneRun a, PlaneRun b, int n_frames, int w, int h,
                      unsigned long long* partials);

constexpr int kSsimTileBW = 32, kSsimTileBH = 8;
inline int ssim_tiles(int w, int h) {
  const int ww = (w >> 2) - 1, wh = (h >> 2) - 1;
  if (ww < 1 || wh < 1) return 0;
  return ((ww + kSsimTileBW - 1) / kSsimTileBW) * ((wh + kSsimTileBH - 1) / kSsimTileBH);
}
hipError_t launch_ssim(hipStream_t stream, Elem elem, PlaneRun main, PlaneRun ref, int n_frames, int w, int h,
                       int max_value, double* partials, unsigned long long* sse_partials);

constexpr int kLumaBlocks = 128;
hipError_t launch_luma_stats(hipStream_t stream, Elem elem, PlaneRun luma, int n_frames, int w, int h,
                             unsigned threshold, int gray_bit_depth, unsigned long long* partials,
                             unsigned long long* out);
void luma_gray_map(int bit_depth, float* a, float* b);

struct FinalizeArgs {
  int n_frames;
  int has_vif, has_adm, has_motion, n_sse_planes, n_ssim_planes;
  const double* vif_part[4];   int vif_tiles[4];
  const long long* vif_fx_part[4];
  const double* adm_part[4];   int adm_tiles[4];   float adm_area[4];
  const long long* adm_fx_part[4];
  int adm_fx_tiles_x[4], adm_fx_top[4], adm_fx_bottom[4], adm_fx_num_shift[4], adm_fx_den_shift[4];
  long long* adm_fx_acc;
  const double* motion_part;   int motion_tiles;   double motion_norm;
  const unsigned long long* motion_fx_part;
  unsigned motion_wh;
  const unsigned long long* sse_part[3];
  const unsigned long long* sse_part_b[3];
  const unsigned long long* sse_tile_part[3];
  int sse_use_a[3];
  const double* ssim_part[3];  int ssim_tiles[3];  double ssim_norm[3];
  double* records;
  int slot_base, slot_step, capacity;
  int record_stride;
};
hipError_t launch_finalize(hipStream_t stream, const FinalizeArgs& args);

constexpr int kSsfTileW = 64, kSsfTileH = 32;
constexpr int kMsScales = 5;
int ssf_tiles(int w, int h);
int ssf_decimation(int w, int h);
hipError_t launch_ssf_map(hipStream_t stream, Elem elem, PlaneRun ref, PlaneRun dis, int n_frames, int src_w, int src_h,
                          int box, float inv_scale, double* partials, MutPlaneRun down_ref = MutPlaneRun{nullptr, 0, 0},
                          MutPlaneRun down_dis = MutPlaneRun{nullptr, 0, 0});
hipError_t launch_ssf_down(hipStream_t stream, Elem elem, PlaneRun ref, PlaneRun dis, int n_frames, int w, int h,
                           float inv_scale, MutPlaneRun out_ref, MutPlaneRun out_dis);
struct SsfFinalizeArgs {
  int n_frames;
  double* ext;
  int ext_stride;
  int slot_base, slot_step, capacity;
  const double* fs_part;   int fs_tiles;   double fs_norm;
  const double* ms_part[kMsScales];   int ms_tiles[kMsScales];   double ms_norm[kMsScales];
};
hipError_t launch_ssf_finalize(hipStream_t stream, const SsfFinalizeArgs& args);
hipError_t launch_ext_fill_nan(hipStream_t stream, double* ext, int slot_base, int n_rows, int capacity, int stride);

constexpr int kCiedeTileW = 64, kCiedeTileH = 4;
int ciede_tiles(int cw, int ch);
hipError_t launch_ciede(hipStream_t stream, Elem elem, const PlaneRun ref[3], const PlaneRun dis[3], int n_frames, int w,
                        int h, int hshift, int vshift, int bit_depth, double* partials);
struct CiedeFinalizeArgs {
  int n_frames;
  double* ext;
  int ext_stride;
  int slot_base, slot_step, capacity;
  const double* partials;
  int n_tiles;
  double norm;
};
hipError_t launch_ciede_finalize(hipStream_t stream, const CiedeFinalizeArgs& args);
hipError_t launch_ciede_debug(hipStream_t stream, const float* lab_pairs, int n, float* de_out);

constexpr int kCambiScales = 5, kCambiDiffs = 4;
constexpr int kCambiParamInts = 22;
struct CambiParams {
  int ws, r, piw, mask_t;
  int tvi[kCambiDiffs];
  int weights[kCambiDiffs];
  int sw[kCambiScales], sh[kCambiScales];
  int64_t off[kCambiScales + 1];
  int chunk[kCambiScales + 1];
  int topk[kCambiScales];
};
CambiParams cambi_params(int w, int h);
hipError_t cambi_prepare(const CambiParams& prm, int bit_depth);
struct CambiWork {
  uint16_t* plane;
  uint8_t* mask;
  float* cmap;
  uint32_t* hist;
  int32_t* sel;
  double* partials;
};
hipError_t launch_cambi(hipStream_t stream, Elem elem, PlaneRun luma, int n_frames, int w, int h, int bit_depth,
                        const CambiParams& prm, const CambiWork& wk, double* ext, int ext_stride, int slot, int slot_base,
                        int slot_step, int capacity);

constexpr int kPhvTileRows = 4;
constexpr int kPhvTableFloats = 384;
struct PsnrHvsGeometry {
  int nbx[3], nby[3], tiles_x[3], tile0[4];
};
void psnr_hvs_geometry(const int pw[3], const int ph[3], PsnrHvsGeometry* g);
void psnr_hvs_tables(float* out);
void psnr_hvs_fdct8x8_host(const int32_t* in, int32_t* out, int n);
hipError_t psnr_hvs_prepare();
hipError_t launch_psnr_hvs(hipStream_t stream, Elem elem, const PlaneRun ref[3], const PlaneRun dis[3], int n_frames,
                           const PsnrHvsGeometry& geo, double* partials, float* block_err = nullptr, int dbg_plane = 0);
struct PsnrHvsFinalizeArgs {
  int n_frames;
  double* ext2;
  int ext_stride;
  int slot_base, slot_step, capacity;
  const double* partials;
// ... 168 lines not shown
```

### pqa2_amd/csrc/pqa_api.hip

```cpp
#include "pqa_ctx.h"

#include <algorithm>
#include <array>
#include <cstdarg>
#include <cstdio>
#include <cstdlib>
#include <mutex>

#include "ingest.h"

using namespace pqa;
using pqa::host::PackPool;
using pqa::host::PackTask;
using pqa::host::run_pack_task;

static thread_local std::string g_create_error;

int pqa::fail(pqa_ctx* c, int code, const char* fmt, ...) {
  char buf[512];
  va_list ap;
  va_start(ap, fmt);
  vsnprintf(buf, sizeof buf, fmt, ap);
  va_end(ap);
  if (c) c->err = buf; else g_create_error = buf;
// ... 122 lines not shown
  int vif_np[4], adm_np[4], motion_np;
  int n_sse = 0, n_ssim = 0;
  bool sse_a[3] = {false, false, false}, sse_b[3] = {false, false, false}, sse_t[3] = {false, false, false};
  int slot(int64_t f) const { return (int)((first + f) % capacity); }
};

int fork_streams(pqa_ctx* c, const Batch& b) {
  HIPCHK(c, hipEventRecord(c->fork_ev, b.st));
  HIPCHK(c, hipStreamWaitEvent(b.st_adm, c->fork_ev, 0));
  HIPCHK(c, hipStreamWaitEvent(b.st_misc, c->fork_ev, 0));
  return PQA_OK;
}

int join_streams(pqa_ctx* c, const Batch& b) {
  HIPCHK(c, hipEventRecord(c->join_ev[0], b.st_adm));
  HIPCHK(c, hipEventRecord(c->join_ev[1], b.st_misc));
  HIPCHK(c, hipStreamWaitEvent(b.st, c->join_ev[0], 0));
  HIPCHK(c, hipStreamWaitEvent(b.st, c->join_ev[1], 0));
  return PQA_OK;
}

struct Scale { int s; Elem elem; RunPair in; int w, h; MutRunPair out; };

template <typename Launch>
int walk_pyramid(const Level (&lv)[4], Scale first, Elem deep, Launch launch) {
  for (Scale k = first; k.s < 4; ++k.s) {
    k.out = k.s < 3 ? level_out(lv[k.s + 1]) : MutRunPair{};
    const int rc = launch(k);
    if (rc != PQA_OK) return rc;
    if (k.s < 3) {
      const Level& L = lv[k.s + 1];
      k.in = level_in(L);
      k.elem = deep;
      k.w = L.w; k.h = L.h;
    }
  }
  return PQA_OK;
}

int hist_alloc(pqa_ctx* c, HistPlane* hp, int p) {
  hp->pitch = round_up((int64_t)c->pw[p] * c->esize, 64);
  return dev_alloc(c, &hp->base, (size_t)hp->pitch * c->ph[p]);
}

int alloc_vif(pqa_ctx* c) {
  const bool on = c->cfg.features & PQA_FEAT_VIF;
  if (on && !c->vif_fixed) HIPCHK(c, vif_march_prepare());
  if (c->vif_fixed) {
    std::vector<uint16_t> lut(32768);
    vif_fixed_log2_table(lut.data());
    PQACHK(dev_alloc(c, &c->vif_lut, lut.size()));
    HIPCHK(c, hipMemcpy(c->vif_lut, lut.data(), lut.size() * sizeof(uint16_t), hipMemcpyHostToDevice));
  }
  int vw = c->pw[0], vh = c->ph[0];
  for (int s = 0; s < 4; ++s) {
    if (s > 0) {
      vw /= 2; vh /= 2;
      Level& V = c->vif_lv[s];
      V.w = vw; V.h = vh; V.pitch = round_up(vw, 16); V.frame_pitch = V.pitch * vh;
      if (on) {
        PQACHK(dev_alloc(c, &V.ref, (size_t)V.frame_pitch * c->B));
        PQACHK(dev_alloc(c, &V.dis, (size_t)V.frame_pitch * c->B));
      }
    }
    if (vw < 2 || vh < 2) return fail(c, PQA_EINVAL, "frame too small for 4 VIF scales");
    c->vif_tiles[s] = vif_tiles_x(s, vw) * vif_tiles_y(vh);
    if (s == 0) {
      const int mp = vif_march_partials_max(vw, vh);
      c->vif_part_cap0 = c->vif_tiles[0] > mp ? c->vif_tiles[0] : mp;
    }
    if (on && !c->vif_fixed)
      PQACHK(dev_alloc(c, &c->vif_part[s], (size_t)(s == 0 ? c->vif_part_cap0 : c->vif_tiles[s]) * 2 * c->B));
    if (on && c->vif_fixed) PQACHK(dev_alloc(c, &c->vif_fx_part[s], (size_t)c->vif_tiles[s] * kVifFxPartials * c->B));
  }
  return PQA_OK;
}

int run_vif(pqa_ctx* c, Batch& b) {
  if (!(c->cfg.features & PQA_FEAT_VIF) || b.sp_n == 0) return PQA_OK;
  const Scale top{0, c->elem, RunPair{b.rs[0], b.ds[0]}, b.w, b.h, {}};
  if (c->vif_fixed)
    return walk_pyramid(c->vif_lv, top, ELEM_U16, [&](const Scale& k) -> int {
      ProfScope ps(c, k.s, b.sp_n, b.st);
      HIPCHK(c, launch_vif_fixed(b.st, k.s, (int)c->cfg.bit_depth, k.elem, k.in.ref, k.in.dis, b.sp_n, k.w, k.h,
                                 c->cfg.vif_enhn_gain_limit, c->vif_lut, c->vif_fx_part[k.s], k.out.ref, k.out.dis));
      return PQA_OK;
    });
  return walk_pyramid(c->vif_lv, top, ELEM_F32, [&](const Scale& k) -> int {
    {
      ProfScope ps(c, k.s, b.sp_n, b.st);
      HIPCHK(c, launch_vif_stat(b.st, k.s, k.elem, k.in.ref, k.in.dis, b.sp_n, k.w, k.h, c->inv_scale,
                                (float)c->cfg.vif_enhn_gain_limit, c->cfg.vif_border == PQA_VIF_BORDER_INTEGER, c->vif_part[k.s],
                                k.out.ref, k.out.dis, c->vif_s0_mode, &b.vif_np[k.s], c->vif_uniform,
                                (c->vif_strip_mask >> k.s & 1) ? c->vif_strip_seg : -1));
    }
    return k.s == 0 && b.fork_late ? fork_streams(c, b) : PQA_OK;
  });
}

int alloc_adm(pqa_ctx* c) {
  const bool on = c->cfg.features & PQA_FEAT_ADM;
  const int w = c->pw[0], h = c->ph[0], B = c->B;
  if (c->adm_fixed) {
    std::vector<int32_t> lut(65537);
    adm_fixed_div_table(lut.data());
    PQACHK(dev_alloc(c, &c->adm_div_lut, lut.size()));
    HIPCHK(c, hipMemcpy(c->adm_div_lut, lut.data(), lut.size() * sizeof(int32_t), hipMemcpyHostToDevice));
    PQACHK(dev_alloc(c, &c->adm_fx_acc, (size_t)c->capacity * 24));
    HIPCHK(c, hipMemsetAsync(c->adm_fx_acc, 0, (size_t)c->capacity * 24 * sizeof(long long), c->stream));
  }
  int aw = w, ah = h;
  for (int s = 0; s < 4; ++s) {
    if (s > 0) {
      aw = (aw + 1) / 2; ah = (ah + 1) / 2;
      Level& A = c->adm_lv[s];
      A.w = aw; A.h = ah; A.pitch = round_up(aw, 16); A.frame_pitch = A.pitch * ah;
      if (on) {
        PQACHK(dev_alloc(c, &A.ref, (size_t)A.frame_pitch * B));
        PQACHK(dev_alloc(c, &A.dis, (size_t)A.frame_pitch * B));
      }
    }
    const int bw = (aw + 1) / 2, bh = (ah + 1) / 2;
    c->adm_tiles[s] = adm_tiles_x(bw) * adm_tiles_y(bh);
    const int left = (int)(bw * 0.1 - 0.5), top = (int)(bh * 0.1 - 0.5);
    c->adm_area[s] = (float)((bh - 2 * top) * (bw - 2 * left));
    c->adm_fx[s] = adm_fixed_scale_params(s, bw, bh);
    if (on && !c->adm_fixed) {
      int mp = adm_march_partials(bw, bh);
      if (s < 2 && adm_pyramid_takes(c->elem, w, h)) { const int pp = adm_pyramid_partials(w, h); mp = pp > mp ? pp : mp; }
      PQACHK(dev_alloc(c, &c->adm_part[s], (size_t)(c->adm_tiles[s] > mp ? c->adm_tiles[s] : mp) * 6 * B));
    }
    if (on && c->adm_fixed) PQACHK(dev_alloc(c, &c->adm_fx_part[s], (size_t)c->adm_tiles[s] * kAdmFxRows * 6 * B));
  }
  return PQA_OK;
}

int run_adm(pqa_ctx* c, Batch& b) {
  if (!(c->cfg.features & PQA_FEAT_ADM) || b.sp_n == 0) return PQA_OK;
  Scale top{0, c->elem, RunPair{b.rs[0], b.ds[0]}, b.w, b.h, {}};
  if (c->adm_fixed)
    return walk_pyramid(c->adm_lv, top, ELEM_F32, [&](const Scale& k) -> int {
      ProfScope ps(c, 7 + k.s, b.sp_n, b.st_adm);
      HIPCHK(c, launch_adm_fixed(b.st_adm, k.s, (int)c->cfg.bit_depth, k.elem, k.in.ref, k.in.dis, b.sp_n, k.w, k.h,
                                 c->cfg.adm_enhn_gain_limit, c->adm_div_lut, k.out.ref, k.out.dis, c->adm_fx_part[k.s]));
      return PQA_OK;
    });
  if (c->adm_mode == ADM_AUTO) {
    const Level& L2 = c->adm_lv[2];
    hipError_t perr = hipSuccess;
    int np = 0;
    ProfScope ps(c, 7, b.sp_n, b.st_adm);
    if (launch_adm_pyramid(b.st_adm, top.elem, top.in.ref, top.in.dis, b.sp_n, top.w, top.h, c->inv_scale,
                           (float)c->cfg.adm_enhn_gain_limit, level_out(L2).ref, level_out(L2).dis, c->adm_part[0], c->adm_part[1],
                           &np, &perr)) {
      HIPCHK(c, perr);
      b.adm_np[0] = b.adm_np[1] = np;
      top = Scale{2, ELEM_F32, level_in(L2), L2.w, L2.h, {}};
    }
  }
  return walk_pyramid(c->adm_lv, top, ELEM_F32, [&](const Scale& k) -> int {
    ProfScope ps(c, 7 + k.s, b.sp_n, b.st_adm);
    HIPCHK(c, launch_adm_scale(b.st_adm, k.s, k.elem, k.in.ref, k.in.dis, b.sp_n, k.w, k.h, c->inv_scale,
                               (float)c->cfg.adm_enhn_gain_limit, k.out.ref, k.out.dis, c->adm_part[k.s], c->adm_mode, &b.adm_np[k.s]));
    return PQA_OK;
  });
}

struct History { uint32_t feature; host::FrameChain* chain; const HistPlane* planes; bool dis; int np; };
std::array<History, 5> histories(pqa_ctx* c) {
  return {{{PQA_FEAT_MOTION, &c->mo_chain, &c->mo_hist, false, 1},
           {PQA_FEAT_XPSNR, &c->xp_chain, c->xp_hist, false, 1},
           {PQA_FEAT_SITI, &c->st_chain[0], &c->st_hist[0], true, 1},
           {PQA_FEAT_SITI, &c->st_chain[1], &c->st_hist[1], false, 1},
           {PQA_FEAT_INTEGRITY, &c->ig_chain, c->ig_hist, true, c->n_planes}}};
}

Pred held(const host::FrameChain& chain, const HistPlane* planes, int64_t frame, int es) {
  const int j = chain.find(frame);
  return j < 0 ? Pred{} : Pred{planes[j].base, planes[j].pitch / es};
}

int alloc_motion(pqa_ctx* c) {
  const int w = c->pw[0], h = c->ph[0];
  c->motion_tiles_n = motion_tiles(w, h);
  if (!(c->cfg.features & PQA_FEAT_MOTION)) return PQA_OK;
  const int mp = motion_march_partials(w, h);
  PQACHK(dev_alloc(c, &c->motion_part, (size_t)(c->motion_tiles_n > mp ? c->motion_tiles_n : mp) * c->B));
  if (c->motion_fixed) PQACHK(dev_alloc(c, &c->motion_fx_part, (size_t)c->motion_tiles_n * c->B));
  return hist_alloc(c, &c->mo_hist, 0);
}

int run_motion(pqa_ctx* c, Batch& b) {
  if (!(c->cfg.features & PQA_FEAT_MOTION)) return PQA_OK;
  const Pred p0 = b.prev.base ? b.prev : held(c->mo_chain, &c->mo_hist, b.first - 1, b.es);
  ProfScope ps(c, 11, b.n, b.st_misc);
  if (c->motion_fixed)
    HIPCHK(c, launch_motion_fixed(b.st_misc, (int)c->cfg.bit_depth, c->elem, b.r[0], p0.base, p0.pitch, b.n, b.w, b.h,
                                  c->motion_fx_part));
  else
    HIPCHK(c, launch_motion(b.st_misc, c->elem, b.r[0], p0.base, p0.pitch, b.n, b.w, b.h, c->inv_scale, c->motion_part,
                            c->motion_mode, &b.motion_np));
  return PQA_OK;
}

int alloc_psnr_ssim(pqa_ctx* c) {
  const uint32_t feat = c->cfg.features;
  for (int p = 0; p < c->n_planes; ++p) {
    if (feat & PQA_FEAT_PSNR) {
      PQACHK(dev_alloc(c, &c->sse_part[p], (size_t)kSseBlocksPerPlane * c->B));
      PQACHK(dev_alloc(c, &c->sse_part_b[p], (size_t)kSseBlocksPerPlane * c->B));
    }
    if (feat & PQA_FEAT_SSIM) {
      c->ssim_tiles_n[p] = ssim_tiles(c->pw[p], c->ph[p]);
      const int ww = (c->pw[p] >> 2) - 1, wh = (c->ph[p] >> 2) - 1;
      c->ssim_norm[p] = (ww > 0 && wh > 0) ? 1.0 / ((double)ww * wh) : 0.0;
      PQACHK(dev_alloc(c, &c->ssim_part[p], (size_t)(c->ssim_tiles_n[p] ? c->ssim_tiles_n[p] : 1) * c->B));
      PQACHK(dev_alloc(c, &c->sse_tile_part[p], (size_t)(c->ssim_tiles_n[p] ? c->ssim_tiles_n[p] : 1) * c->B));
    }
  }
  return PQA_OK;
}

int run_psnr_ssim(pqa_ctx* c, Batch& b) {
  const uint32_t feat = c->cfg.features;
  const int es = b.es;
  const bool both = (feat & PQA_FEAT_PSNR) && (feat & PQA_FEAT_SSIM);
  if (feat & PQA_FEAT_PSNR) {
    b.n_sse = c->n_planes;
    ProfScope ps(c, 12, b.n, b.st_misc);
    for (int p = 0; p < c->n_planes; ++p) {
      const PlaneRun a = b.d[p], r = b.r[p];
      const int pw = c->pw[p], ph = c->ph[p];
      if (both && c->ssim_tiles_n[p] > 0) {
        b.sse_t[p] = true;
        const int w4 = (pw >> 2) << 2, h4 = (ph >> 2) << 2;
        if (w4 < pw) {
          HIPCHK(c, launch_sse(b.st_misc, c->elem, run_at(a, w4, es), run_at(r, w4, es), b.n, pw - w4, ph, c->sse_part[p]));
          b.sse_a[p] = true;
        }
        if (h4 < ph) {
          HIPCHK(c, launch_sse(b.st_misc, c->elem, run_at(a, h4 * a.row_pitch, es), run_at(r, h4 * r.row_pitch, es), b.n, w4,
                               ph - h4, c->sse_part_b[p]));
          b.sse_b[p] = true;
        }
      } else {
        HIPCHK(c, launch_sse(b.st_misc, c->elem, a, r, b.n, pw, ph, c->sse_part[p]));
        b.sse_a[p] = true;
      }
    }
  }
  if (feat & PQA_FEAT_SSIM) {
    b.n_ssim = c->n_planes;
    ProfScope ps(c, 13, b.n, b.st_misc);
    for (int p = 0; p < c->n_planes; ++p)
      HIPCHK(c, launch_ssim(b.st_misc, c->elem, b.d[p], b.r[p], b.n, c->pw[p], c->ph[p], (1 << c->cfg.bit_depth) - 1,
                            c->ssim_part[p], b.sse_t[p] ? c->sse_tile_part[p] : nullptr));
  }
  return PQA_OK;
}

int alloc_rings(pqa_ctx* c) {
  try {
    c->ring.init(c->capacity);
  } catch (...) {
    return fail(c, PQA_ENOMEM, "out of host memory");
  }
  PQACHK(dev_alloc(c, &c->luma_part, (size_t)kLumaBlocks * 3 * c->B));
  PQACHK(dev_alloc(c, &c->luma_out, (size_t)3 * (c->B > kLumaOutFrames ? c->B : kLumaOutFrames)));
  PQACHK(dev_alloc(c, &c->records, (size_t)c->capacity * PQA_RECORD_DOUBLES));
  for (int i = 0; i < kExtBlocks; ++i) {
    if (!(c->cfg.features & kExtBlock[i].features)) continue;
    PQACHK(dev_alloc(c, &c->ext[i], (size_t)c->capacity * kExtBlock[i].doubles));
    HIPCHK(c, launch_ext_fill_nan(c->stream, c->ext[i], 0, c->capacity, c->capacity, kExtBlock[i].doubles));
  }
  HIPCHK(c, hipMemsetAsync(c->records, 0, (size_t)c->capacity * PQA_RECORD_DOUBLES * sizeof(double), c->stream));
  HIPCHK(c, hipStreamSynchronize(c->stream));
  return PQA_OK;
}

int fill_ext_nan(pqa_ctx* c, Batch& b) {
  for (int i = 0; b.k > 1 && i < kExtBlocks; ++i)
    if (kExtBlock[i].spatial && c->ext[i])
      HIPCHK(c, launch_ext_fill_nan(b.st_misc, c->ext[i], b.slot(0), b.n, c->capacity, kExtBlock[i].doubles));
  return PQA_OK;
}

int alloc_ssim_family(pqa_ctx* c) {
  const uint32_t feat = c->cfg.features;
  const int w = c->pw[0], h = c->ph[0], B = c->B;
  size_t per_frame = 0;
  int sw = w, sh = h;
  for (int j = 0; j < kMsScales; ++j) {
    Level& L = c->ms_lv[j];
    L.w = sw; L.h = sh;
    if (j > 0) { L.pitch = round_up(sw, 16); L.frame_pitch = L.pitch * sh; per_frame += (size_t)L.frame_pitch * 2 * sizeof(float); }
    c->ms_tiles[j] = ssf_tiles(sw, sh);
    sw = (sw + 1) / 2; sh = (sh + 1) / 2;
  }
  c->ssf_sb = B;
  if ((feat & PQA_FEAT_MS_SSIM) && per_frame) {
    const int64_t sb = (int64_t)(320ll << 20) / (int64_t)per_frame;
    c->ssf_sb = (int)(sb < 1 ? 1 : sb < B ? sb : B);
  }
  const int SB = c->ssf_sb;
  for (int j = 0; (feat & PQA_FEAT_MS_SSIM) && j < kMsScales; ++j) {
    Level& L = c->ms_lv[j];
    if (j > 0) {
      PQACHK(dev_alloc(c, &L.ref, (size_t)L.frame_pitch * SB));
      PQACHK(dev_alloc(c, &L.dis, (size_t)L.frame_pitch * SB));
    }
    PQACHK(dev_alloc(c, &c->ms_part[j], (size_t)c->ms_tiles[j] * 4 * SB));
  }
  if (feat & PQA_FEAT_FLOAT_SSIM) {
    c->fs_box = ssf_decimation(w, h);
    c->fs_tiles = ssf_tiles((w + c->fs_box - 1) / c->fs_box, (h + c->fs_box - 1) / c->fs_box);
    PQACHK(dev_alloc(c, &c->fs_part, (size_t)c->fs_tiles * 4 * SB));
// ... 455 lines not shown
      return fail(c, PQA_ESTATE, "more pending frames than result_capacity %d", c->capacity);
    rc = staging_half_ready(c, c->cur_half);
    if (rc != PQA_OK) return rc;
    Half& H = c->half[c->cur_half];
    if (c->pending == 0) {
      c->pending_first = frame_index;
      if (H.copied_pending) {
        HIPCHK(c, hipEventSynchronize(H.copied));
        H.copied_pending = false;
      }
      if (H.computed_pending) {
        HIPCHK(c, hipStreamWaitEvent(c->copy_stream, H.computed, 0));
        H.computed_pending = false;
      }
    }
    const int slot0 = c->pending;
    bool ok = true;
    hipError_t copy_err = hipSuccess;
    const auto upload = [&](int k) {
      const size_t off = (size_t)(slot0 + k) * c->slot_bytes;
      copy_err = hipMemcpyAsync(H.dev + off, H.pinned + off, c->slot_bytes, hipMemcpyHostToDevice, c->copy_stream);
      return copy_err == hipSuccess;
    };
    try {
      c->pack_tasks.clear();
      static const unsigned task_bytes = [] { const char* e = getenv("PQA_PACK_TASK_KB"); const int kb = e ? atoi(e) : 0; return (unsigned)(kb > 0 ? kb : 1024) << 10; }();
      for (int k = 0; k < m; ++k) {
        uint8_t* slot = H.pinned + (size_t)(slot0 + k) * c->slot_bytes;
        for (int side = 0; side < 2; ++side)
          for (int p = 0; p < c->n_planes; ++p) {
            const PlaneSrc& ps = src[side][p];
            const int64_t step = (int64_t)(done + k) * frame_step[side];
            const size_t row_bytes = (size_t)c->pw[p] * c->esize;
            int rows_per = (int)(task_bytes / (row_bytes ? row_bytes : 1));
            if (rows_per < 1) rows_per = 1;
            for (int y = 0; y < c->ph[p]; y += rows_per) {
              const int rows = c->ph[p] - y < rows_per ? c->ph[p] - y : rows_per;
              PackTask t{slot + c->plane_off[side][p] + (int64_t)y * c->slot_row_pitch[p],
                         ps.fd < 0 ? ps.ptr + step + (int64_t)y * ps.stride : nullptr, c->slot_row_pitch[p], ps.stride, row_bytes, rows};
              t.fd = ps.fd;
              t.file_off = ps.off + step + (int64_t)y * ps.stride;
              t.frame = k;
              c->pack_tasks.push_back(t);
            }
          }
      }
      if (c->slot_bytes >= (4u << 20)) ensure_pack_pool(c);
      if (c->pack_pool && c->slot_bytes >= (4u << 20)) {
        ok = c->pack_pool->run_frames(c->pack_tasks.data(), (int)c->pack_tasks.size(), m, upload);
      } else {
        int k_done = 0;
        for (size_t i = 0; i < c->pack_tasks.size() && ok; ++i) {
          ok = run_pack_task(c->pack_tasks[i]);
          if (ok && (i + 1 == c->pack_tasks.size() || c->pack_tasks[i + 1].frame != c->pack_tasks[i].frame)) ok = upload(k_done++);
        }
      }
    } catch (...) {
      return fail(c, PQA_ENOMEM, "out of host memory while staging frame %lld", (long long)frame_index);
    }
    if (copy_err != hipSuccess) return fail(c, PQA_EDEVICE, "hipMemcpyAsync failed: %s", hipGetErrorString(copy_err));
    if (!ok)
      return fail(c, PQA_EINVAL, "frame %lld%s: short read from a file source (truncated file or bad plane offset)",
                  (long long)frame_index, m > 1 ? " (or one of the frames after it in this run)" : "");
    c->pending += m;
    done += m;
    if (c->pending == c->HB) {
      rc = flush_pending(c);
      if (rc != PQA_OK) return rc;
    }
  }
  return PQA_OK;
}

int submit_one(pqa_ctx* c, int64_t frame_index, const PlaneSrc (&src)[2][3]) {
  const int64_t no_step[2] = {0, 0};
  return submit_run(c, frame_index, 1, src, no_step);
}

int check_config(const pqa_config* cfg) {
  if (cfg->struct_size != sizeof(pqa_config)) return fail(nullptr, PQA_EINVAL, "pqa_config.struct_size mismatch");
  if (cfg->width < 16 || cfg->height < 16 || cfg->width > 16384 || cfg->height > 16384)
    return fail(nullptr, PQA_EINVAL, "unsupported frame size %ux%u (16..16384)", cfg->width, cfg->height);
  if (cfg->bit_depth != 8 && cfg->bit_depth != 10 && cfg->bit_depth != 12)
    return fail(nullptr, PQA_EINVAL, "unsupported bit depth %u (8, 10, 12)", cfg->bit_depth);
  if (cfg->n_planes != 1 && cfg->n_planes != 3) return fail(nullptr, PQA_EINVAL, "n_planes must be 1 or 3");
  if (cfg->chroma_hshift > 2 || cfg->chroma_vshift > 2) return fail(nullptr, PQA_EINVAL, "bad chroma shift");
  if ((cfg->features & ~(uint32_t)PQA_FEAT_KNOWN) || cfg->features == 0)
    return fail(nullptr, PQA_EINVAL, "bad feature mask 0x%x", cfg->features);
  if (cfg->features & PQA_FEAT_FLOAT_SSIM) {
    const int f = ssf_decimation((int)cfg->width, (int)cfg->height);
    if (ssf_tiles(((int)cfg->width + f - 1) / f, ((int)cfg->height + f - 1) / f) == 0)
      return fail(nullptr, PQA_EINVAL, "frame %ux%u too small for float_ssim (decimated by %d it must be >= 11x11)", cfg->width,
                  cfg->height, f);
  }
  if (cfg->features & PQA_FEAT_MS_SSIM) {
    int sw = (int)cfg->width, sh = (int)cfg->height;
    for (int j = 1; j < kMsScales; ++j) { sw = (sw + 1) / 2; sh = (sh + 1) / 2; }
    if (ssf_tiles(sw, sh) == 0)
      return fail(nullptr, PQA_EINVAL, "frame %ux%u too small for float_ms_ssim (5th scale %dx%d, needs >= 11x11: w, h >= 161)",
                  cfg->width, cfg->height, sw, sh);
  }
  if ((cfg->features & PQA_FEAT_CIEDE) && cfg->n_planes != 3)
    return fail(nullptr, PQA_EINVAL, "ciede2000 needs the chroma planes: n_planes must be 3 (got %u)", cfg->n_planes);
  if ((cfg->features & PQA_FEAT_CAMBI_FULL_REF) && !(cfg->features & PQA_FEAT_CAMBI))
    return fail(nullptr, PQA_EINVAL, "cambi full reference (PQA_FEAT_CAMBI_FULL_REF) needs PQA_FEAT_CAMBI");
  if ((cfg->features & PQA_FEAT_CAMBI) && cfg->bit_depth != 8 && cfg->bit_depth != 10)
    return fail(nullptr, PQA_EINVAL, "cambi supports bit depth 8 or 10 (got %u)", cfg->bit_depth);
  if ((cfg->features & PQA_FEAT_PSNR_HVS) && cfg->n_planes != 3)
    return fail(nullptr, PQA_EINVAL, "psnr_hvs needs the chroma planes: n_planes must be 3 (got %u)", cfg->n_planes);
  if ((cfg->features & PQA_FEAT_PSNR_HVS) &&
      (((cfg->width + (1u << cfg->chroma_hshift) - 1) >> cfg->chroma_hshift) < 8 ||
       ((cfg->height + (1u << cfg->chroma_vshift) - 1) >> cfg->chroma_vshift) < 8))
    return fail(nullptr, PQA_EINVAL, "psnr_hvs needs every plane >= 8x8 (frame %ux%u, chroma shifts %u, %u)", cfg->width,
                cfg->height, cfg->chroma_hshift, cfg->chroma_vshift);
  if ((cfg->features & PQA_FEAT_XPSNR_HFR) && !(cfg->features & PQA_FEAT_XPSNR))
    return fail(nullptr, PQA_EINVAL, "xpsnr second-order term (PQA_FEAT_XPSNR_HFR) needs PQA_FEAT_XPSNR");
  if (cfg->features & PQA_FEAT_XPSNR) {
    XpsnrGeometry g{};
    xpsnr_geometry((int)cfg->width, (int)cfg->height, (int)((cfg->width + (1u << cfg->chroma_hshift) - 1) >> cfg->chroma_hshift),
                   (int)((cfg->height + (1u << cfg->chroma_vshift) - 1) >> cfg->chroma_vshift), (int)cfg->n_planes,
                   (int)cfg->bit_depth, &g);
    if (g.bv == 2 && ((cfg->width | cfg->height) & 1))
      return fail(nullptr, PQA_EINVAL, "xpsnr needs an even width and height above 2048x1152 (its 2x2 activity; got %ux%u)",
                  cfg->width, cfg->height);
    if (g.nc_blk > g.n_blk || (cfg->n_planes == 3 && g.nc_blk == 0) || g.bsx + 4 > kXpLdsCols)
      return fail(nullptr, PQA_EINVAL, "xpsnr: unsupported block grid for %ux%u (chroma shifts %u, %u)", cfg->width,
                  cfg->height, cfg->chroma_hshift, cfg->chroma_vshift);
  }
  if ((cfg->features & (PQA_FEAT_SITI_REF_FULL | PQA_FEAT_SITI_DIS_FULL)) && !(cfg->features & PQA_FEAT_SITI))
    return fail(nullptr, PQA_EINVAL, "siti range bits (PQA_FEAT_SITI_REF_FULL / _DIS_FULL) need PQA_FEAT_SITI");
  if ((cfg->features & PQA_FEAT_SITI) && cfg->bit_depth != 8 && cfg->bit_depth != 10)
    return fail(nullptr, PQA_EINVAL, "siti supports bit depth 8 or 10 (got %u)", cfg->bit_depth);
  if (cfg->vif_border > PQA_VIF_BORDER_INTEGER || (cfg->fixed_point & ~(uint32_t)PQA_FIXED_ALL))
    return fail(nullptr, PQA_EINVAL, "bad vif_border %u / fixed_point 0x%x", cfg->vif_border, cfg->fixed_point);
  return PQA_OK;
}

void read_switches(pqa_ctx* c) {
  const char* e = getenv("PQA_MULTI_STREAM");
  c->multi_stream = (e && e[0] == '1') ? 1 : (e && e[0] == '2') ? 2 : 0;
  const char* t = getenv("PQA_TRACE");
  c->trace = t && t[0] == '1';
  const char* v = getenv("PQA_VIF_MFMA");
  c->vif_s0_mode = (v && v[0] == '0') ? VIF_S0_VALU : VIF_S0_AUTO;
  const char* vu = getenv("PQA_VIF_UNIFORM");
  c->vif_uniform = !(vu && vu[0] == '0');
  const char* vs = getenv("PQA_VIF_STRIP");
  if (vs && vs[0]) c->vif_strip_mask = atoi(vs) & 0xe;
  const char* vg = getenv("PQA_VIF_STRIP_SEG");
  c->vif_strip_seg = vg ? std::max(0, atoi(vg)) : 0;
  const char* am = getenv("PQA_ADM_MARCH");
  const char* ap = getenv("PQA_ADM_PYRAMID");
  c->adm_mode = (am && am[0] == '0') ? ADM_TILED : (ap && ap[0] == '0') ? ADM_MARCH : ADM_AUTO;
  const char* mm = getenv("PQA_MOTION_MARCH");
  c->motion_mode = (mm && mm[0] == '0') ? MOTION_TILED : MOTION_AUTO;
  const char* xm = getenv("PQA_XSSE_MFMA");
  c->xsse_mfma = !(xm && xm[0] == '0');
  const char* tw = getenv("PQA_TEMPORAL_WALK");
  c->temporal_walk = tw && tw[0] == '1';
}

int create_streams(pqa_ctx* c) {
  HIPCHK(c, hipSetDevice(c->device));
  HIPCHK(c, hipStreamCreateWithFlags(&c->own_stream, hipStreamNonBlocking));
  c->stream = c->own_stream;
  for (int i = 0; i < 2; ++i) {
    HIPCHK(c, hipStreamCreateWithFlags(&c->aux[i], hipStreamNonBlocking));
    HIPCHK(c, hipEventCreateWithFlags(&c->join_ev[i], hipEventDisableTiming));
  }
  HIPCHK(c, hipEventCreateWithFlags(&c->fork_ev, hipEventDisableTiming));
  for (int i = 0; i < kBatchEvents; ++i) HIPCHK(c, hipEventCreateWithFlags(&c->batch_ev[i], hipEventDisableTiming));
  return PQA_OK;
}

}

extern "C" {

const char* pqa_version(void) { return "pqa_vmaf 0.2.0 (gfx950; libvmaf-float VIF/ADM/motion, FFmpeg psnr/ssim; VIF scale 0 on the f16 matrix cores)"; }
int pqa_record_doubles(void) { return PQA_RECORD_DOUBLES; }
int pqa_ext_doubles(void) { return PQA_EXT_DOUBLES; }
int pqa_ext2_doubles(void) { return PQA_EXT2_DOUBLES; }
int pqa_ext3_doubles(void) { return PQA_EXT3_DOUBLES; }
int pqa_ext4_doubles(void) { return PQA_EXT4_DOUBLES; }
int pqa_ext5_doubles(void) { return PQA_EXT5_DOUBLES; }

void pqa_config_init(pqa_config* cfg, uint32_t width, uint32_t height) {
  if (!cfg) return;
  memset(cfg, 0, sizeof *cfg);
  cfg->struct_size = sizeof *cfg;
  cfg->width = width; cfg->height = height;
  cfg->bit_depth = 8;
  cfg->n_planes = 1;
  cfg->chroma_hshift = cfg->chroma_vshift = 1;
  cfg->features = PQA_FEAT_VMAF;
  cfg->max_batch = 0;
  cfg->result_capacity = 16384;
  cfg->n_subsample = 1;
  cfg->vif_enhn_gain_limit = 100.0;
  cfg->adm_enhn_gain_limit = 100.0;
}

int pqa_create(const pqa_config* cfg, pqa_ctx** out) {
  if (!cfg || !out) return fail(nullptr, PQA_EINVAL, "null argument");
  *out = nullptr;
  PQACHK(check_config(cfg));
  int ndev = 0;
  if (hipGetDeviceCount(&ndev) != hipSuccess || ndev <= 0)
    return fail(nullptr, PQA_EDEVICE, "no HIP device visible (this library has no CPU fallback)");
  if (cfg->device < 0 || cfg->device >= ndev) return fail(nullptr, PQA_EINVAL, "device %d out of range (%d)", cfg->device, ndev);

  pqa_ctx* c = new (std::nothrow) pqa_ctx();
  if (!c) return fail(nullptr, PQA_ENOMEM, "out of host memory");
  c->cfg = *cfg;
  c->device = cfg->device;
  if (cfg->max_batch) {
    c->B = (int)cfg->max_batch;
  } else {
    const int64_t per_frame = 2ll * cfg->width * cfg->height * (cfg->bit_depth > 8 ? 2 : 1);
    c->B = (int)((1536ll << 20) / per_frame);
    if (c->B < 8) c->B = 8;
  }
  if (c->B > 256) c->B = 256;
  c->HB = c->B < 8 ? c->B : 8;
  c->capacity = cfg->result_capacity ? (int)cfg->result_capacity : 16384;
  if (c->capacity < c->B) c->capacity = c->B;
  c->k_sub = cfg->n_subsample > 1 ? (int)cfg->n_subsample : 1;
  if (c->cfg.vif_enhn_gain_limit <= 0) c->cfg.vif_enhn_gain_limit = 100.0;
  if (c->cfg.adm_enhn_gain_limit <= 0) c->cfg.adm_enhn_gain_limit = 100.0;
  c->elem = cfg->bit_depth > 8 ? ELEM_U16 : ELEM_U8;
  c->esize = cfg->bit_depth > 8 ? 2 : 1;
  c->inv_scale = 1.0f / (float)(1 << (cfg->bit_depth - 8));
  c->n_planes = (int)cfg->n_planes;
  c->pw[0] = (int)cfg->width; c->ph[0] = (int)cfg->height;
  for (int p = 1; p < 3; ++p) {
    c->pw[p] = (int)((cfg->width + (1u << cfg->chroma_hshift) - 1) >> cfg->chroma_hshift);
    c->ph[p] = (int)((cfg->height + (1u << cfg->chroma_vshift) - 1) >> cfg->chroma_vshift);
  }
  c->vif_fixed = (cfg->features & PQA_FEAT_VIF) && (cfg->fixed_point & PQA_FIXED_VIF);
  c->motion_fixed = (cfg->features & PQA_FEAT_MOTION) && (cfg->fixed_point & PQA_FIXED_MOTION);
  c->adm_fixed = (cfg->features & PQA_FEAT_ADM) && (cfg->fixed_point & PQA_FIXED_ADM);
  const double f = (double)(1 << (cfg->bit_depth - 8));
  c->black_thr = (uint32_t)(16.0 * f + 0.10 * 219.0 * f);
  read_switches(c);
  static const struct { uint32_t features; int (*make)(pqa_ctx*); } kParts[] = {
      {0, create_streams}, {0, alloc_vif}, {0, alloc_adm}, {0, alloc_motion}, {0, alloc_psnr_ssim},
      {PQA_FEAT_FLOAT_SSIM | PQA_FEAT_MS_SSIM, alloc_ssim_family}, {PQA_FEAT_CIEDE, alloc_ciede}, {PQA_FEAT_CAMBI, alloc_cambi},
      {PQA_FEAT_PSNR_HVS, alloc_psnr_hvs}, {PQA_FEAT_XPSNR, alloc_xpsnr}, {PQA_FEAT_SITI, alloc_siti},
      {PQA_FEAT_INTEGRITY, alloc_integrity}, {0, alloc_rings}};
  for (const auto& part : kParts) {
    if (part.features && !(cfg->features & part.features)) continue;
    if (const int rc = part.make(c); rc != PQA_OK) {
      g_create_error = c->err;
      pqa_destroy(c);
      return rc;
    }
  }
  *out = c;
  return PQA_OK;
}

void pqa_destroy(pqa_ctx* c) {
  if (!c) return;
  if (c->pin_thread.joinable()) c->pin_thread.join();
  hipSetDevice(c->device);
  if (c->stream) hipStreamSynchronize(c->stream);
  if (c->copy_stream) hipStreamSynchronize(c->copy_stream);
  if (c->pk_stream) hipStreamSynchronize(c->pk_stream);
  for (int i = 0; i < 2; ++i) if (c->aux[i]) hipStreamSynchronize(c->aux[i]);
  prof_drain(c);
  for (void* p : c->allocs) hipFree(p);
  {
    StagingSet mine;
    mine.device = c->device;
    mine.bytes = c->slot_bytes * (size_t)c->HB;
    bool complete = c->staging_ready;
    for (int i = 0; i < 2; ++i) {
      mine.pinned[i] = c->half[i].pinned;
      mine.dev[i] = c->half[i].dev;
      complete = complete && mine.pinned[i] && mine.dev[i];
    }
    if (complete && staging_cache_enabled()) {
      std::lock_guard<std::mutex> g(g_staging_mu);
      if (g_staging.bytes) {
        if (g_staging.device != c->device) hipSetDevice(g_staging.device);
        staging_release(g_staging);
        hipSetDevice(c->device);
      }
      g_staging = mine;
    } else {
      staging_release(mine);
    }
  }
  for (int i = 0; i < 2; ++i) {
    Half& H = c->half[i];
    if (H.copied) hipEventDestroy(H.copied);
    if (H.computed) hipEventDestroy(H.computed);
  }
  for (int i = 0; i < 2; ++i) {
    Half& L = c->luma_half[i];
    if (L.pinned) hipHostFree(L.pinned);
    if (L.dev) hipFree(L.dev);
    if (L.copied) hipEventDestroy(L.copied);
  }
  for (int i = 0; i < 2; ++i) {
    for (int sd = 0; sd < 2; ++sd) {
// ... 702 lines not shown
```

### pqa2_amd/csrc/pqa_ctx.h

```cpp
#pragma once
#include "../../include/pqa_vmaf.h"

#include <atomic>
#include <cstring>
#include <memory>
#include <string>
#include <thread>
#include <vector>

#include "host_chain.h"
#include "host_pack.h"
#include "host_ring.h"
#include "host_packed.h"
#include "host_stage.h"
#include "kernels.h"

namespace pqa {

struct Level {
  int w = 0, h = 0;
  int64_t pitch = 0, frame_pitch = 0;
  float* ref = nullptr;
  float* dis = nullptr;
};
// ... 27 lines not shown
    {PQA_EXT5_DOUBLES, PQA_FEAT_INTEGRITY, false},
};

constexpr int kLumaOutFrames = 2048;

enum SideBuf {
  SIDE_XSSE_PART = 0, SIDE_XSSE_NORM_REF, SIDE_XSSE_NORM_DIS, SIDE_XSSE_OUT,
  SIDE_XSSE_REF, SIDE_XSSE_DIS,
  SIDE_SHIFT_PART, SIDE_SHIFT_ROWSQ, SIDE_SHIFT_OUT,
  SIDE_LEVEL_OUT,
  SIDE_RS_TABLE0, SIDE_RS_TABLE1, SIDE_RS_TABLE2, SIDE_RS_TABLE3,
  SIDE_RS_SRC, SIDE_RS_DST,
  SIDE_PAIR_REF, SIDE_PAIR_DIS,
  SIDE_FLOW_OUT,
  SIDE_COLOUR_A, SIDE_COLOUR_B, SIDE_COLOUR_OUT,
  SIDE_PROF_SRC, SIDE_PROF_OUT,
  SIDE_TILE_OUT,
  SIDE_BAND_PART, SIDE_BAND_OUT,
  SIDE_TEMPORAL_OUT,
  SIDE_EDGE_OUT,
  SIDE_UNPACK_SRC, SIDE_UNPACK_DST,
  SIDE_CONVERT_SRC, SIDE_CONVERT_DST,
  kSideBufs
};

constexpr int kRsCached = 4;
struct RsCached {
  bool valid = false;
  pqa_resample_spec spec{};
  ResamplePlan plan;
};

}

struct pqa_ctx {
  pqa_config cfg{};
  int device = 0;
  hipStream_t own_stream = nullptr, stream = nullptr, copy_stream = nullptr;
  hipStream_t aux[2] = {nullptr, nullptr};
  hipEvent_t fork_ev = nullptr, join_ev[2] = {nullptr, nullptr};
  pqa::Elem elem = pqa::ELEM_U8;
  int esize = 1;
  float inv_scale = 1.0f;
  int pw[3] = {0, 0, 0}, ph[3] = {0, 0, 0};
  int n_planes = 1;
  int B = 8, HB = 8, capacity = 16384, k_sub = 1;
  pqa::Level vif_lv[4], adm_lv[4];
  double* vif_part[4] = {};
  long long* vif_fx_part[4] = {};
  uint16_t* vif_lut = nullptr;
  bool vif_fixed = false, motion_fixed = false, adm_fixed = false;
  long long* adm_fx_part[4] = {};
  long long* adm_fx_acc = nullptr;
  int32_t* adm_div_lut = nullptr;
  pqa::AdmFxScale adm_fx[4] = {};
  unsigned long long* motion_fx_part = nullptr;
  int vif_tiles[4] = {};
  int vif_part_cap0 = 0;
  double* adm_part[4] = {};
  int adm_tiles[4] = {};
  float adm_area[4] = {};
  double* motion_part = nullptr;
  int motion_tiles_n = 0;
  unsigned long long* sse_part[3] = {};
  unsigned long long* sse_part_b[3] = {};
  unsigned long long* sse_tile_part[3] = {};
  double* ssim_part[3] = {};
  int ssim_tiles_n[3] = {};
  double ssim_norm[3] = {};
  double* records = nullptr;
  double* ext[pqa::kExtBlocks] = {};
  pqa::Level ms_lv[pqa::kMsScales];
  double* ms_part[pqa::kMsScales] = {};
  int ms_tiles[pqa::kMsScales] = {};
  double* fs_part = nullptr;
  int fs_tiles = 0, fs_box = 1;
  int ssf_sb = 0;
  double* ciede_part = nullptr;
  int ciede_tiles_n = 0;
  pqa::CambiParams cambi_prm{};
  pqa::CambiWork cambi_wk{};
  int cambi_sb = 0;
  pqa::PsnrHvsGeometry phv_geo{};
  double* phv_part = nullptr;
  pqa::XpsnrGeometry xp_geo{};
  unsigned long long* xp_blk = nullptr;
  double* xp_w = nullptr;
  pqa::HistPlane xp_hist[2];
  pqa::host::FrameChain xp_chain{2};
  uint8_t* xp_prev = nullptr;
  double* st_part = nullptr;
  pqa::HistPlane st_hist[2];
  pqa::host::FrameChain st_chain[2];
  unsigned long long* ig_part = nullptr;
  pqa::HistPlane ig_hist[3];
  pqa::host::FrameChain ig_chain;
  uint32_t black_thr = 0;
  bool started = false;
  uint8_t* ig_anchor[3] = {nullptr, nullptr, nullptr};
  uint8_t* ig_stage = nullptr;
  size_t ig_stage_off[3] = {0, 0, 0}, ig_stage_bytes = 0;
  unsigned long long* ig_out = nullptr;
  unsigned long long* luma_part = nullptr;
  unsigned long long* luma_out = nullptr;
  pqa::Half luma_half[2];
  int64_t luma_pitch = 0;
  int LB = 0;
  bool luma_ready = false;
  uint32_t luma_gray = PQA_GRAY_LUMA;
  bool xsse_mfma = true;
  bool temporal_walk = false;
  pqa::RsCached rs_cache[pqa::kRsCached];
  int rs_next = 0;
  uint8_t* side_pin[2] = {nullptr, nullptr};
  size_t side_pin_cap[2] = {0, 0};
  void* side_buf[pqa::kSideBufs] = {};
  size_t side_cap[pqa::kSideBufs] = {};
  pqa::HistPlane mo_hist;
  pqa::host::FrameChain mo_chain;
  pqa::Half half[2];
  int cur_half = 0, pending = 0;
  int64_t pending_first = 0;
  size_t slot_bytes = 0;
  size_t plane_off[2][3] = {};
  int64_t slot_row_pitch[3] = {};
  bool staging_ready = false;
  std::thread pin_thread;
  hipError_t pin_err = hipSuccess;
  uint8_t* surf_dev = nullptr;
  uint8_t* pk_pin[2][2] = {};
  uint8_t* pk_dev[2][2] = {};
  size_t pk_pin_cap[2][2] = {}, pk_dev_cap[2][2] = {};
  hipStream_t pk_stream = nullptr;
  hipEvent_t pk_copied[2] = {nullptr, nullptr}, pk_computed[2] = {nullptr, nullptr};
  bool pk_copied_pending[2] = {false, false}, pk_computed_pending[2] = {false, false};
  int pk_set = 0;
  std::unique_ptr<pqa::host::PackPool> pack_pool;
  bool pack_pool_tried = false;
  std::vector<pqa::host::PackTask> pack_tasks;
  pqa::host::RecordRing ring;
  hipEvent_t batch_ev[pqa::kBatchEvents] = {};
  uint64_t batch_ev_seq[pqa::kBatchEvents] = {};
  uint64_t batch_seq = 0;
  uint64_t done_seq = 0;
  std::atomic<int> cancelled{0};
  std::string err;
  std::vector<void*> allocs;
  int multi_stream = 0;
  int vif_s0_mode = pqa::VIF_S0_AUTO;
  int vif_uniform = 1;
  int vif_strip_mask = 0x2;
  int vif_strip_seg = 0;
  int adm_mode = pqa::ADM_AUTO;
  int motion_mode = pqa::MOTION_AUTO;
  bool trace = false;
  bool prof = false;
  uint32_t prof_mask = 0xffffffffu;
  std::vector<pqa::ProfEv> evs;
  double prof_ms[PQA_PROF_KERNELS] = {};
  uint64_t prof_n[PQA_PROF_KERNELS] = {}, prof_frames[PQA_PROF_KERNELS] = {};
};

namespace pqa {

int fail(pqa_ctx* c, int code, const char* fmt, ...);

#define HIPCHK(c, expr)                                                                          \
  do {                                                                                           \
    hipError_t e_ = (expr);                                                                      \
    if (e_ != hipSuccess)                                                                        \
      return pqa::fail((c), e_ == hipErrorOutOfMemory ? PQA_ENOMEM : PQA_EDEVICE, "%s failed: %s", #expr, \
                  hipGetErrorString(e_));                                                        \
  } while (0)

#define PQACHK(expr)                   \
  do {                                 \
    const int rc_ = (expr);            \
    if (rc_ != PQA_OK) return rc_;     \
  } while (0)

template <typename T>
int dev_alloc(pqa_ctx* c, T** out, size_t count) {
  void* p = nullptr;
  if (count == 0) count = 1;
  HIPCHK(c, hipMalloc(&p, count * sizeof(T)));
  c->allocs.push_back(p);
  *out = (T*)p;
  return PQA_OK;
}

}
```

### pqa2_amd/csrc/pqa_debug.hip

```cpp
#include "pqa_ctx.h"

using namespace pqa;

namespace {

int need_device() {
  int ndev = 0;
  if (hipGetDeviceCount(&ndev) != hipSuccess || ndev <= 0)
    return fail(nullptr, PQA_EDEVICE, "no HIP device visible (this library has no CPU fallback)");
  return PQA_OK;
}

int plane_pitch_rule(const char* who, uint32_t bit_depth, uint32_t w, int64_t row_pitch_bytes, int* es) {
  *es = bit_depth > 8 ? 2 : 1;
  if (row_pitch_bytes < (int64_t)w * *es || row_pitch_bytes % *es)
    return fail(nullptr, PQA_EINVAL, "%s: bad row pitch %lld", who, (long long)row_pitch_bytes);
  return PQA_OK;
}

struct Scratch {
  void* held[12];
  int n = 0;
  hipError_t err = hipSuccess;
  ~Scratch() { for (int i = 0; i < n; ++i) hipFree(held[i]); }
  template <typename T>
  T* get(size_t count) {
    void* p = nullptr;
    if (err == hipSuccess) err = n < 12 ? hipMalloc(&p, count * sizeof(T)) : hipErrorOutOfMemory;
    if (p) held[n++] = p;
    return (T*)p;
  }
  void* plane(const void* host, int64_t row_pitch_bytes, size_t row_bytes, uint32_t h) {
    if (!host) return nullptr;
    void* p = get<uint8_t>(row_bytes * h);
    if (err == hipSuccess) err = hipMemcpy2D(p, row_bytes, host, (size_t)row_pitch_bytes, row_bytes, h, hipMemcpyHostToDevice);
    return p;
  }
};

}

extern "C" {

int pqa_debug_vif_march_table(uint16_t* out, int32_t capacity_halfwords) { return vif_march_table(out, capacity_halfwords); }
int pqa_debug_vif_march_shape(uint32_t width, uint32_t height, int32_t* out6) {
  if (!out6 || width == 0 || height == 0 || width > 65536 || height > 65536) return PQA_EINVAL;
  int shape[6];
  vif_march_shape((int)width, (int)height, shape);
  for (int i = 0; i < 6; ++i) out6[i] = shape[i];
  return PQA_OK;
}

int pqa_debug_vif_strip_shape(pqa_ctx* ctx, uint32_t scale, uint32_t n_frames, int32_t* out4) {
  if (!ctx) return PQA_EINVAL;
  if (!out4 || scale < 1 || scale > 3 || n_frames == 0 || n_frames > 65536)
    return fail(ctx, PQA_EINVAL, "pqa_debug_vif_strip_shape: bad argument");
  const Level& L = ctx->vif_lv[scale];
  int shape[4];
  const int strip_seg = ctx->vif_fixed ? -1 : (ctx->vif_strip_mask >> scale & 1) ? ctx->vif_strip_seg : -1;
  vif_strip_shape((int)scale, L.w, L.h, (int)n_frames, strip_seg, shape);
  for (int i = 0; i < 4; ++i) out4[i] = shape[i];
  return PQA_OK;
}

int pqa_debug_ciede2000(const double* lab_pairs, int32_t n, double* de_out) {
  if (n < 0 || (n > 0 && (!lab_pairs || !de_out))) return fail(nullptr, PQA_EINVAL, "bad argument");
  const int rc = need_device();
  if (rc != PQA_OK) return rc;
  if (n == 0) return PQA_OK;
  std::vector<float> in((size_t)n * 6), out((size_t)n);
  for (size_t i = 0; i < in.size(); ++i) in[i] = (float)lab_pairs[i];
  Scratch s;
  float* d_in = s.get<float>(in.size());
  float* d_out = s.get<float>(out.size());
  hipError_t e = s.err;
  if (e == hipSuccess) e = hipMemcpy(d_in, in.data(), in.size() * sizeof(float), hipMemcpyHostToDevice);
  if (e == hipSuccess) e = launch_ciede_debug(nullptr, d_in, n, d_out);
  if (e == hipSuccess) e = hipMemcpy(out.data(), d_out, out.size() * sizeof(float), hipMemcpyDeviceToHost);
  if (e != hipSuccess) return fail(nullptr, PQA_EDEVICE, "pqa_debug_ciede2000: %s", hipGetErrorString(e));
  for (int32_t i = 0; i < n; ++i) de_out[i] = (double)out[i];
  return PQA_OK;
}

int pqa_debug_cambi_params(uint32_t w, uint32_t h, uint32_t bit_depth, int32_t* out, int32_t cap) {
  if (!out || cap < PQA_CAMBI_PARAM_INTS) return fail(nullptr, PQA_EINVAL, "pqa_debug_cambi_params: null or short output");
  if (w < 16 || h < 16 || w > 16384 || h > 16384 || (bit_depth != 8 && bit_depth != 10))
    return fail(nullptr, PQA_EINVAL, "pqa_debug_cambi_params: unsupported %ux%u at %u bit", w, h, bit_depth);
  static_assert(kCambiParamInts == PQA_CAMBI_PARAM_INTS, "pqa_debug_cambi_params layout");
  const CambiParams p = cambi_params((int)w, (int)h);
  int i = 0;
  out[i++] = p.ws; out[i++] = p.r; out[i++] = p.piw; out[i++] = p.mask_t;
  for (int d = 0; d < kCambiDiffs; ++d) out[i++] = p.tvi[d];
  for (int d = 0; d < kCambiDiffs; ++d) out[i++] = p.weights[d];
  for (int s = 0; s < kCambiScales; ++s) { out[i++] = p.sw[s]; out[i++] = p.sh[s]; }
  return PQA_OK;
}

int pqa_debug_cambi_cmap(const void* luma, int64_t row_pitch_bytes, uint32_t w, uint32_t h, uint32_t bit_depth, float* cmap,
                         int64_t cap, double* score) {
  if (!luma || !cmap || w < 16 || h < 16 || w > 16384 || h > 16384 || (bit_depth != 8 && bit_depth != 10))
    return fail(nullptr, PQA_EINVAL, "pqa_debug_cambi_cmap: bad argument");
  int es = 1;
  int rc = plane_pitch_rule("pqa_debug_cambi_cmap", bit_depth, w, row_pitch_bytes, &es);
  if (rc != PQA_OK) return rc;
  const CambiParams p = cambi_params((int)w, (int)h);
  const int64_t total = p.off[kCambiScales];
  if (cap < total) return fail(nullptr, PQA_EINVAL, "pqa_debug_cambi_cmap: cmap holds %lld floats, needs %lld", (long long)cap,
                               (long long)total);
  if ((rc = need_device()) != PQA_OK) return rc;
  Scratch s;
  s.err = cambi_prepare(p, (int)bit_depth);
  void* src = s.plane(luma, row_pitch_bytes, (size_t)w * es, h);
  double* ext = s.get<double>(PQA_EXT_DOUBLES);
  CambiWork wk{};
  wk.plane = s.get<uint16_t>((size_t)total);
  wk.mask = s.get<uint8_t>((size_t)total);
  wk.cmap = s.get<float>((size_t)total);
  wk.hist = s.get<uint32_t>((size_t)kCambiScales * 2048);
  wk.sel = s.get<int32_t>((size_t)kCambiScales * 4);
  wk.partials = s.get<double>((size_t)p.chunk[kCambiScales]);
  hipError_t e = s.err;
  if (e == hipSuccess) {
    const PlaneRun run{src, (int64_t)w, (int64_t)w * h};
    e = launch_cambi(nullptr, es == 1 ? ELEM_U8 : ELEM_U16, run, 1, (int)w, (int)h, (int)bit_depth, p, wk, ext, PQA_EXT_DOUBLES,
                     PQA_EXT_CAMBI, 0, 1, 1);
  }
  if (e == hipSuccess) e = hipMemcpy(cmap, wk.cmap, (size_t)total * sizeof(float), hipMemcpyDeviceToHost);
  double ext_row[PQA_EXT_DOUBLES];
  if (e == hipSuccess) e = hipMemcpy(ext_row, ext, sizeof ext_row, hipMemcpyDeviceToHost);
  if (e != hipSuccess) return fail(nullptr, PQA_EDEVICE, "pqa_debug_cambi_cmap: %s", hipGetErrorString(e));
  if (score) *score = ext_row[PQA_EXT_CAMBI];
  return PQA_OK;
}

int pqa_debug_psnr_hvs_dct8x8(const int32_t* in, int32_t* out, int32_t n) {
  if (!in || !out || n < 0) return fail(nullptr, PQA_EINVAL, "pqa_debug_psnr_hvs_dct8x8: bad argument");
  psnr_hvs_fdct8x8_host(in, out, n);
  return PQA_OK;
}

int pqa_debug_psnr_hvs_tables(float* out, int32_t cap) {
  static_assert(kPhvTableFloats == PQA_PSNR_HVS_TABLE_FLOATS, "pqa_debug_psnr_hvs_tables layout");
  if (!out || cap < PQA_PSNR_HVS_TABLE_FLOATS)
    return fail(nullptr, PQA_EINVAL, "pqa_debug_psnr_hvs_tables: null or short output");
  psnr_hvs_tables(out);
  return PQA_OK;
}

int pqa_debug_psnr_hvs_plane(const void* ref, const void* dis, int64_t row_pitch_bytes, uint32_t w, uint32_t h,
                             uint32_t bit_depth, uint32_t plane_kind, float* block_err, double* mse) {
  if (!ref || !dis || !block_err || w < 8 || h < 8 || w > 16384 || h > 16384 || plane_kind > 2 ||
      (bit_depth != 8 && bit_depth != 10 && bit_depth != 12))
    return fail(nullptr, PQA_EINVAL, "pqa_debug_psnr_hvs_plane: bad argument");
  int es = 1;
  int rc = plane_pitch_rule("pqa_debug_psnr_hvs_plane", bit_depth, w, row_pitch_bytes, &es);
  if (rc == PQA_OK) rc = need_device();
  if (rc != PQA_OK) return rc;
  const int pw[3] = {(int)w, (int)w, (int)w}, ph[3] = {(int)h, (int)h, (int)h};
  PsnrHvsGeometry geo{};
  psnr_hvs_geometry(pw, ph, &geo);
  const int nb = geo.nbx[0] * geo.nby[0];
  Scratch s;
  s.err = psnr_hvs_prepare();
  void* src = s.plane(ref, row_pitch_bytes, (size_t)w * es, h);
  void* dst = s.plane(dis, row_pitch_bytes, (size_t)w * es, h);
  double* part = s.get<double>((size_t)geo.tile0[3]);
  double* ext2 = s.get<double>(PQA_EXT2_DOUBLES);
  float* err = s.get<float>((size_t)nb);
  hipError_t e = s.err;
  if (e == hipSuccess) {
    PlaneRun r3[3], d3[3];
    for (int p = 0; p < 3; ++p) {
      r3[p] = PlaneRun{src, (int64_t)w, (int64_t)w * h};
      d3[p] = PlaneRun{dst, (int64_t)w, (int64_t)w * h};
    }
    e = launch_psnr_hvs(nullptr, es == 1 ? ELEM_U8 : ELEM_U16, r3, d3, 1, geo, part, err, (int)plane_kind);
  }
  if (e == hipSuccess) {
    PsnrHvsFinalizeArgs pa{};
    pa.n_frames = 1;
    pa.ext2 = ext2;
    pa.ext_stride = PQA_EXT2_DOUBLES;
    pa.slot_base = 0; pa.slot_step = 1; pa.capacity = 1;
    pa.partials = part;
    for (int p = 0; p < 4; ++p) pa.tile0[p] = geo.tile0[p];
    for (int p = 0; p < 3; ++p) pa.blocks[p] = nb;
    pa.peak = (double)((1 << bit_depth) - 1);
    e = launch_psnr_hvs_finalize(nullptr, pa);
  }
  if (e == hipSuccess) e = hipMemcpy(block_err, err, (size_t)nb * sizeof(float), hipMemcpyDeviceToHost);
  double row[PQA_EXT2_DOUBLES];
  if (e == hipSuccess) e = hipMemcpy(row, ext2, sizeof row, hipMemcpyDeviceToHost);
  if (e != hipSuccess) return fail(nullptr, PQA_EDEVICE, "pqa_debug_psnr_hvs_plane: %s", hipGetErrorString(e));
  if (mse) *mse = row[PQA_EXT2_PSNR_HVS_MSE + plane_kind];
  return PQA_OK;
}

int pqa_debug_xpsnr_blocks(const void* ref, const void* ref_m1, const void* ref_m2, const void* dis, int64_t row_pitch_bytes,
                           uint32_t w, uint32_t h, uint32_t bit_depth, int32_t hfr, uint64_t* out, double* wsse) {
  if (!ref || !dis || !out || w < 16 || h < 16 || w > 16384 || h > 16384 ||
      (bit_depth != 8 && bit_depth != 10 && bit_depth != 12))
    return fail(nullptr, PQA_EINVAL, "pqa_debug_xpsnr_blocks: bad argument");
  int es = 1;
  int rc = plane_pitch_rule("pqa_debug_xpsnr_blocks", bit_depth, w, row_pitch_bytes, &es);
  if (rc != PQA_OK) return rc;
  XpsnrGeometry geo{};
  xpsnr_geometry((int)w, (int)h, (int)w, (int)h, 1, (int)bit_depth, &geo);
  if (geo.bv == 2 && ((w | h) & 1)) return fail(nullptr, PQA_EINVAL, "pqa_debug_xpsnr_blocks: odd size above 2048x1152");
  if ((rc = need_device()) != PQA_OK) return rc;
  Scratch s;
  const void* host[4] = {ref, ref_m1, ref_m2, dis};
  void* dev[4];
  for (int i = 0; i < 4; ++i) dev[i] = s.plane(host[i], row_pitch_bytes, (size_t)w * es, h);
  auto* blk = s.get<unsigned long long>((size_t)geo.n_blk * kXpBlockVals);
// ... 118 lines not shown
```

Measured before the change: 22410 frames/s.

## Restrict ADM pyramid LL output to the dependency cone of scored windows

```diff
diff --git a/include/pqa_vmaf.h b/include/pqa_vmaf.h
--- a/include/pqa_vmaf.h
+++ b/include/pqa_vmaf.h
@@ -393,6 +393,8 @@
 
 PQA_API int pqa_debug_vif_strip_shape(pqa_ctx* ctx, uint32_t scale, uint32_t n_frames, int32_t* out4);
 
+PQA_API int pqa_debug_adm_need(uint32_t width, uint32_t height, int32_t* out20);
+
 PQA_API int pqa_debug_ciede2000(const double* lab_pairs, int32_t n, double* de_out);
 
 enum { PQA_CAMBI_PARAM_INTS = 22 };
diff --git a/pqa2_amd/_native.py b/pqa2_amd/_native.py
--- a/pqa2_amd/_native.py
+++ b/pqa2_amd/_native.py
@@ -54,7 +54,7 @@
     "pqa_submit", "pqa_submit_fd", "pqa_submit_fd_run", "pqa_submit_device", "pqa_submit_surfaces", "pqa_submit_packed", "pqa_set_motion_halo", "pqa_set_ref_history", "pqa_set_dis_history", "pqa_set_dis_history_planes", "pqa_set_black_threshold", "pqa_frame_sad", "pqa_frame_sad_device", "pqa_flush", "pqa_collect", "pqa_collect_ext", "pqa_collect_ext2", "pqa_collect_ext3", "pqa_collect_ext4", "pqa_collect_ext5", "pqa_sync",
     "pqa_cancel", "pqa_reset", "pqa_last_error", "pqa_luma_stats_device", "pqa_luma_stats", "pqa_cross_sse_device", "pqa_cross_sse", "pqa_shift_sse_device", "pqa_shift_sse", "pqa_level_stats_device", "pqa_level_stats", "pqa_level_bins", "pqa_resample", "pqa_resample_device", "pqa_unpack", "pqa_unpack_device", "pqa_format_convert", "pqa_format_convert_device", "pqa_flow_moments", "pqa_flow_moments_device", "pqa_line_profiles", "pqa_line_profiles_device", "pqa_tile_moments", "pqa_tile_moments_device", "pqa_band_moments", "pqa_band_moments_device", "pqa_band_sums", "pqa_temporal_moments", "pqa_temporal_moments_device", "pqa_temporal_sums", "pqa_edge_profiles", "pqa_edge_profiles_device", "pqa_edge_sums", "pqa_colour_sums", "pqa_colour_moments", "pqa_colour_moments_device", "pqa_colour_apply", "pqa_colour_apply_device", "pqa_set_luma_gray",
     "pqa_profile_enable",
-    "pqa_profile_read", "pqa_profile_kernel_name", "pqa_debug_vif_march_table", "pqa_debug_vif_march_shape", "pqa_debug_vif_strip_shape",
+    "pqa_profile_read", "pqa_profile_kernel_name", "pqa_debug_vif_march_table", "pqa_debug_vif_march_shape", "pqa_debug_vif_strip_shape", "pqa_debug_adm_need",
     "pqa_debug_ciede2000", "pqa_debug_cambi_params", "pqa_debug_cambi_cmap", "pqa_debug_psnr_hvs_dct8x8",
     "pqa_debug_psnr_hvs_tables", "pqa_debug_psnr_hvs_plane", "pqa_debug_xpsnr_blocks", "pqa_debug_siti_plane",
     "pqa_debug_resample_table", "pqa_debug_colour",
@@ -295,6 +295,7 @@
     lib.pqa_debug_vif_march_table.argtypes = [vp, i32]
     lib.pqa_debug_vif_march_shape.argtypes = [C.c_uint32, C.c_uint32, C.POINTER(i32 * 6)]
     lib.pqa_debug_vif_strip_shape.argtypes = [vp, C.c_uint32, C.c_uint32, C.POINTER(i32 * 4)]
+    lib.pqa_debug_adm_need.argtypes = [C.c_uint32, C.c_uint32, C.POINTER(i32 * 20)]
     lib.pqa_debug_ciede2000.argtypes = [vp, i32, vp]
     lib.pqa_debug_cambi_params.argtypes = [C.c_uint32, C.c_uint32, C.c_uint32, vp, i32]
     lib.pqa_debug_cambi_cmap.argtypes = [vp, C.c_int64, C.c_uint32, C.c_uint32, C.c_uint32, vp, C.c_int64, vp]
diff --git a/pqa2_amd/csrc/adm.hip b/pqa2_amd/csrc/adm.hip
--- a/pqa2_amd/csrc/adm.hip
+++ b/pqa2_amd/csrc/adm.hip
@@ -274,13 +274,13 @@
 
 hipError_t launch_adm_scale(hipStream_t stream, int scale, Elem elem, PlaneRun ref, PlaneRun dis, int n_frames,
                             int w, int h, float inv_scale, float gain_limit, MutPlaneRun ll_ref,
-                            MutPlaneRun ll_dis, double* partials, int mode, int* n_partials) {
+                            MutPlaneRun ll_dis, double* partials, int mode, int* n_partials, bool cone) {
   if (n_partials) *n_partials = adm_tiles_x((w + 1) / 2) * adm_tiles_y((h + 1) / 2);
   if (n_frames <= 0) return hipSuccess;
   if (mode != ADM_TILED) {
     hipError_t err = hipSuccess;
     if (launch_adm_march(stream, scale, elem, ref, dis, n_frames, w, h, inv_scale, gain_limit, ll_ref, ll_dis, partials,
-                         n_partials, &err))
+                         n_partials, cone, &err))
       return err;
   }
   AdmArgs a{};
diff --git a/pqa2_amd/csrc/adm_march.hip b/pqa2_amd/csrc/adm_march.hip
--- a/pqa2_amd/csrc/adm_march.hip
+++ b/pqa2_amd/csrc/adm_march.hip
@@ -1,6 +1,7 @@
 #include <type_traits>
 
 #include "adm_chain.h"
+#include "adm_need.h"
 #include "kernels.h"
 #include "pqa_device.h"
 
@@ -22,6 +23,7 @@
   int left, top, right, bottom;
   int reg_start[4];
   int seg_rows[3], seg_first[4];
+  int need_r0, need_r1, need_c0, need_c1;
   float inv_scale, gain_limit, rf_hv, rf_d, k_hv, k_d;
   float* ll_ref;
   float* ll_dis;
@@ -228,11 +230,13 @@
   const int stripe = sg * 4 + wave;
   double* __restrict__ part = a.partials + ((int64_t)fr * a.n_part + (int64_t)id * 4 + wave) * 6;
   const int region = seg >= a.seg_first[2] ? 2 : seg >= a.seg_first[1] ? 1 : 0;
-  const int r0 = a.reg_start[region] + (seg - a.seg_first[region]) * a.seg_rows[region];
-  const int r1 = min(r0 + a.seg_rows[region], a.reg_start[region + 1]);
+  int r0 = a.reg_start[region] + (seg - a.seg_first[region]) * a.seg_rows[region];
+  int r1 = min(r0 + a.seg_rows[region], a.reg_start[region + 1]);
+  if (region != 1) { r0 = max(r0, a.need_r0); r1 = min(r1, a.need_r1); }
   const int cs = stripe * kStripe;
   const bool in_win = region == 1 && cs < a.right && cs + kStripe > a.left;
-  if (stripe >= a.n_stripes || (!in_win && !a.ll_ref)) {
+  const bool owed = a.ll_ref && r0 < r1 && cs < a.need_c1 && cs + kStripe > a.need_c0;
+  if (stripe >= a.n_stripes || (!in_win && !owed)) {
     if (lane < 6) part[lane] = 0.0;
     return;
   }
@@ -241,7 +245,7 @@
   float* __restrict__ ll_r = a.ll_ref ? a.ll_ref + (int64_t)fr * a.ll_frame_pitch_r : nullptr;
   float* __restrict__ ll_d = a.ll_ref ? a.ll_dis + (int64_t)fr * a.ll_frame_pitch_d : nullptr;
   const int c = cs - kHalo + lane;
-  const unsigned ll_voff = (lane >= kHalo && lane < kHalo + kStripe && c < a.ow) ? (unsigned)c * 4u : 0x80000000u;
+  const unsigned ll_voff = (lane >= kHalo && lane < kHalo + kStripe && c >= a.need_c0 && c < a.need_c1) ? (unsigned)c * 4u : 0x80000000u;
   const bool fast = a.aligned && cs >= kHalo && 2 * (cs + kStripe + kHalo - 1) + 1 < a.w;
   const unsigned bytes_r = (unsigned)a.h * a.pitch_r * (unsigned)sizeof(T), bytes_d = (unsigned)a.h * a.pitch_d * (unsigned)sizeof(T);
   if (fast) {
@@ -305,7 +309,7 @@
 
 bool launch_adm_march(hipStream_t stream, int scale, Elem elem, PlaneRun ref, PlaneRun dis, int n_frames, int w, int h,
                       float inv_scale, float gain_limit, MutPlaneRun ll_ref, MutPlaneRun ll_dis, double* partials,
-                      int* n_partials, hipError_t* err) {
+                      int* n_partials, bool cone, hipError_t* err) {
   const int es = elem == ELEM_U8 ? 1 : elem == ELEM_U16 ? 2 : 4;
   if ((int64_t)ref.row_pitch * h * es >= (1ll << 31) || (int64_t)dis.row_pitch * h * es >= (1ll << 31)) return false;
   AdmMarchArgs a{};
@@ -328,6 +332,9 @@
   const Partition p = partition_rows(a.oh, a.top, a.bottom, a.n_stripes);
   for (int r = 0; r < 4; ++r) { a.reg_start[r] = p.reg_start[r]; a.seg_first[r] = p.seg_first[r]; }
   for (int r = 0; r < 3; ++r) a.seg_rows[r] = p.seg_rows[r];
+  AdmSpan need_rows, need_cols;
+  adm_need_scale(scale, w, h, cone, &need_rows, &need_cols);
+  a.need_r0 = need_rows.lo; a.need_r1 = need_rows.hi; a.need_c0 = need_cols.lo; a.need_c1 = need_cols.hi;
   a.inv_scale = inv_scale; a.gain_limit = gain_limit;
   a.rf_hv = 1.0f / adm_dwt_quant_step(scale, 1);
   a.rf_d = 1.0f / adm_dwt_quant_step(scale, 2);
diff --git a/pqa2_amd/csrc/adm_need.h b/pqa2_amd/csrc/adm_need.h
--- /dev/null
+++ b/pqa2_amd/csrc/adm_need.h
@@ -0,0 +1,51 @@
+#pragma once
+
+namespace pqa {
+
+struct AdmSpan {
+  int lo, hi;
+};
+struct AdmNeed {
+  AdmSpan rows[4], cols[4];
+  AdmSpan in_rows, in_cols;
+};
+
+inline void adm_need_axis(int n, int n_scales, bool cone, AdmSpan* need, AdmSpan* input) {
+  int len[4];
+  for (int s = 0, m = n; s < n_scales; ++s) { m = (m + 1) / 2; len[s] = m; }
+  AdmSpan above{0, 0};
+  for (int s = n_scales - 1; s >= 0; --s) {
+    const int lo_win = (int)(len[s] * 0.1 - 0.5);
+    AdmSpan r{lo_win - 1, len[s] - lo_win + 1};
+    if (s < n_scales - 1) {
+      const int a = 2 * above.lo - 1, b = 2 * above.hi + 1;
+      r.lo = a < r.lo ? a : r.lo;
+      r.hi = b > r.hi ? b : r.hi;
+    }
+    if (!cone) r = AdmSpan{0, len[s]};
+    r.lo = r.lo < 0 ? 0 : r.lo;
+    r.hi = r.hi > len[s] ? len[s] : r.hi;
+    need[s] = above = r;
+  }
+  AdmSpan in{2 * above.lo - 1, 2 * above.hi + 1};
+  in.lo = in.lo < 0 ? 0 : in.lo;
+  in.hi = in.hi > n ? n : in.hi;
+  *input = in;
+}
+
+inline AdmNeed adm_need(int w, int h, bool cone = true) {
+  AdmNeed o{};
+  adm_need_axis(h, 4, cone, o.rows, &o.in_rows);
+  adm_need_axis(w, 4, cone, o.cols, &o.in_cols);
+  return o;
+}
+
+inline void adm_need_scale(int scale, int w, int h, bool cone, AdmSpan* rows, AdmSpan* cols) {
+  AdmSpan need[4], in;
+  adm_need_axis(h, 4 - scale, cone, need, &in);
+  *rows = need[0];
+  adm_need_axis(w, 4 - scale, cone, need, &in);
+  *cols = need[0];
+}
+
+}
diff --git a/pqa2_amd/csrc/adm_pyramid.hip b/pqa2_amd/csrc/adm_pyramid.hip
--- a/pqa2_amd/csrc/adm_pyramid.hip
+++ b/pqa2_amd/csrc/adm_pyramid.hip
@@ -1,6 +1,7 @@
 #include <type_traits>
 
 #include "adm_chain.h"
+#include "adm_need.h"
 #include "kernels.h"
 #include "pqa_device.h"
 
@@ -22,6 +23,7 @@
   int n_stripes, n_sg, seg_rows, n_seg;
   int n_frames;
   int left0, top0, right0, bottom0, left1, top1, right1, bottom1;
+  int nr0, nr1, nc0, nc1;
   float inv_scale;
   Consts k0, k1;
   float* ll_ref;
@@ -109,7 +111,7 @@
   float* __restrict__ ll_d = a.ll_dis + (int64_t)fr * a.ll_frame_pitch_d;
   const rsrc_t ll_rs_r = make_rsrc(ll_r, (unsigned)a.oh1 * a.ll_pitch_r * 4u);
   const rsrc_t ll_rs_d = make_rsrc(ll_d, (unsigned)a.oh1 * a.ll_pitch_d * 4u);
-  const unsigned ll_voff = (inner && c1 < a.ow1) ? (unsigned)c1 * 4u : 0x80000000u;
+  const unsigned ll_voff = (inner && c1 >= a.nc0 && c1 < a.nc1) ? (unsigned)c1 * 4u : 0x80000000u;
 
   float accA[6] = {0, 0, 0, 0, 0, 0}, accB[6] = {0, 0, 0, 0, 0, 0}, acc1[6] = {0, 0, 0, 0, 0, 0};
   const int tid = threadIdx.x;
@@ -195,7 +197,9 @@
     return r;
   };
 
-  const int j_first = R0 - 1, j_last = R1 < a.oh1 ? R1 : R1 - 1;
+  const int Ra = max(R0, a.nr0), Rb = min(R1, a.nr1);
+  const int j_seg = R0 - 1;
+  const int j_first = j_seg + ((Ra - R0) & ~1), j_last = Rb < R1 ? Rb - 1 : R1 < a.oh1 ? R1 : R1 - 1;
   const int i0 = 2 * j_first - 1;
   Row4 x0, x1, x2, x3;
   x2 = ld.convert(ld.load(2 * i0 - 1)); x3 = ld.convert(ld.load(2 * i0));
@@ -224,21 +228,21 @@
     w3 = band_edges(step0(x0, x1, x2, x3, ib, need0(ib), accum0(ib), accum0(ib - 1)));
     if (j == 0) w0 = w2;
     if (ib == a.oh0) w3 = w2;
-    step1(w0, w1, w2, w3, j, need1(j), j >= R0 && j < R1, accum1(j), accum1(j - 1));
+    step1(w0, w1, w2, w3, j, need1(j), j >= Ra && j < Rb, accum1(j), accum1(j - 1));
   };
   if constexpr (sizeof(T) == 1) {
     for (int j = j_first; j <= j_last; j += 2) {
       iteration(j, u0, u1, v0, v1);
       if (j + 1 <= j_last) {
         iteration(j + 1, v0, v1, u0, u1);
-        if (((j + 1 - j_first) & 3) == 3) flush();
+        if (((j + 1 - j_seg) & 3) == 3) flush();
       }
     }
   } else {
     for (int j = j_first; j <= j_last; ++j) {
       iteration(j, u0, u1, v0, v1);
       u0 = v0; u1 = v1;
-      if (((j - j_first) & 3) == 3) flush();
+      if (((j - j_seg) & 3) == 3) flush();
     }
   }
   flush();
@@ -274,11 +278,11 @@
   const int stripe = sg * 4 + wave;
   double* __restrict__ part0 = a.part0 + ((int64_t)fr * a.n_part + (int64_t)id * 4 + wave) * 6;
   double* __restrict__ part1 = a.part1 + ((int64_t)fr * a.n_part + (int64_t)id * 4 + wave) * 6;
-  if (stripe >= a.n_stripes) {
+  const int R0 = seg * a.seg_rows, R1 = min(R0 + a.seg_rows, a.oh1);
+  if (stripe >= a.n_stripes || stripe * kP1 >= a.nc1 || (stripe + 1) * kP1 <= a.nc0 || min(R1, a.nr1) <= max(R0, a.nr0)) {
     if (lane < 6) { part0[lane] = 0.0; part1[lane] = 0.0; }
     return;
   }
-  const int R0 = seg * a.seg_rows, R1 = min(R0 + a.seg_rows, a.oh1);
   const T* __restrict__ ref = (const T*)a.ref + (int64_t)fr * a.frame_pitch_r;
   const T* __restrict__ dis = (const T*)a.dis + (int64_t)fr * a.frame_pitch_d;
   const unsigned bytes_r = (unsigned)a.h * a.pitch_r * (unsigned)sizeof(T), bytes_d = (unsigned)a.h * a.pitch_d * (unsigned)sizeof(T);
@@ -313,7 +317,7 @@
 
 bool launch_adm_pyramid(hipStream_t stream, Elem elem, PlaneRun ref, PlaneRun dis, int n_frames, int w, int h, float inv_scale,
                         float gain_limit, MutPlaneRun ll_ref, MutPlaneRun ll_dis, double* partials0, double* partials1,
-                        int* n_partials, hipError_t* err) {
+                        int* n_partials, bool cone, hipError_t* err) {
   if (!adm_pyramid_takes(elem, w, h) || !ll_ref.base || !ll_dis.base) return false;
   const int es = elem == ELEM_U8 ? 1 : 2;
   if ((int64_t)ref.row_pitch * h * es >= (1ll << 31) || (int64_t)dis.row_pitch * h * es >= (1ll << 31)) return false;
@@ -337,6 +341,11 @@
   a.left1 = (int)(a.ow1 * border - 0.5); a.top1 = (int)(a.oh1 * border - 0.5);
   a.right1 = a.ow1 - a.left1; a.bottom1 = a.oh1 - a.top1;
   if (a.top0 < 2 || a.top1 < 2) return false;
+  AdmNeed need = adm_need(w, h, cone);
+  if (need.rows[0].lo < 2 * need.rows[1].lo - 1 || need.rows[0].hi > 2 * need.rows[1].hi + 1 ||
+      need.cols[0].lo < 2 * need.cols[1].lo - 1 || need.cols[0].hi > 2 * need.cols[1].hi + 1)
+    need = adm_need(w, h, false);
+  a.nr0 = need.rows[1].lo; a.nr1 = need.rows[1].hi; a.nc0 = need.cols[1].lo; a.nc1 = need.cols[1].hi;
   a.inv_scale = inv_scale;
   for (int s = 0; s < 2; ++s) {
     Consts& k = s ? a.k1 : a.k0;
diff --git a/pqa2_amd/csrc/kernels.h b/pqa2_amd/csrc/kernels.h
--- a/pqa2_amd/csrc/kernels.h
+++ b/pqa2_amd/csrc/kernels.h
@@ -51,16 +51,17 @@
 enum : int { ADM_TILED = 0, ADM_AUTO = 1, ADM_MARCH = 2 };
 hipError_t launch_adm_scale(hipStream_t stream, int scale, Elem elem, PlaneRun ref, PlaneRun dis, int n_frames,
                             int w, int h, float inv_scale, float gain_limit, MutPlaneRun ll_ref,
-                            MutPlaneRun ll_dis, double* partials, int mode = ADM_AUTO, int* n_partials = nullptr);
+                            MutPlaneRun ll_dis, double* partials, int mode = ADM_AUTO, int* n_partials = nullptr,
+                            bool cone = true);
 int adm_march_partials(int band_w, int band_h);
 bool launch_adm_march(hipStream_t stream, int scale, Elem elem, PlaneRun ref, PlaneRun dis, int n_frames, int w, int h,
                       float inv_scale, float gain_limit, MutPlaneRun ll_ref, MutPlaneRun ll_dis, double* partials,
-                      int* n_partials, hipError_t* err);
+                      int* n_partials, bool cone, hipError_t* err);
 bool adm_pyramid_takes(Elem elem, int w, int h);
 int adm_pyramid_partials(int w, int h);
 bool launch_adm_pyramid(hipStream_t stream, Elem elem, PlaneRun ref, PlaneRun dis, int n_frames, int w, int h, float inv_scale,
                         float gain_limit, MutPlaneRun ll_ref, MutPlaneRun ll_dis, double* partials0, double* partials1,
-                        int* n_partials, hipError_t* err);
+                        int* n_partials, bool cone, hipError_t* err);
 float adm_dwt_quant_step(int lambda, int theta);
 
 constexpr int kAdmFxRows = kAdmTileH + 2;
diff --git a/pqa2_amd/csrc/pqa_api.hip b/pqa2_amd/csrc/pqa_api.hip
--- a/pqa2_amd/csrc/pqa_api.hip
+++ b/pqa2_amd/csrc/pqa_api.hip
@@ -298,7 +298,7 @@
     ProfScope ps(c, 7, b.sp_n, b.st_adm);
     if (launch_adm_pyramid(b.st_adm, top.elem, top.in.ref, top.in.dis, b.sp_n, top.w, top.h, c->inv_scale,
                            (float)c->cfg.adm_enhn_gain_limit, level_out(L2).ref, level_out(L2).dis, c->adm_part[0], c->adm_part[1],
-                           &np, &perr)) {
+                           &np, c->adm_cone, &perr)) {
       HIPCHK(c, perr);
       b.adm_np[0] = b.adm_np[1] = np;
       top = Scale{2, ELEM_F32, level_in(L2), L2.w, L2.h, {}};
@@ -307,7 +307,8 @@
   return walk_pyramid(c->adm_lv, top, ELEM_F32, [&](const Scale& k) -> int {
     ProfScope ps(c, 7 + k.s, b.sp_n, b.st_adm);
     HIPCHK(c, launch_adm_scale(b.st_adm, k.s, k.elem, k.in.ref, k.in.dis, b.sp_n, k.w, k.h, c->inv_scale,
-                               (float)c->cfg.adm_enhn_gain_limit, k.out.ref, k.out.dis, c->adm_part[k.s], c->adm_mode, &b.adm_np[k.s]));
+                               (float)c->cfg.adm_enhn_gain_limit, k.out.ref, k.out.dis, c->adm_part[k.s], c->adm_mode, &b.adm_np[k.s],
+                               c->adm_cone));
     return PQA_OK;
   });
 }
@@ -1069,6 +1070,8 @@
   const char* am = getenv("PQA_ADM_MARCH");
   const char* ap = getenv("PQA_ADM_PYRAMID");
   c->adm_mode = (am && am[0] == '0') ? ADM_TILED : (ap && ap[0] == '0') ? ADM_MARCH : ADM_AUTO;
+  const char* ac = getenv("PQA_ADM_CONE");
+  c->adm_cone = !(ac && ac[0] == '0');
   const char* mm = getenv("PQA_MOTION_MARCH");
   c->motion_mode = (mm && mm[0] == '0') ? MOTION_TILED : MOTION_AUTO;
   const char* xm = getenv("PQA_XSSE_MFMA");
diff --git a/pqa2_amd/csrc/pqa_ctx.h b/pqa2_amd/csrc/pqa_ctx.h
--- a/pqa2_amd/csrc/pqa_ctx.h
+++ b/pqa2_amd/csrc/pqa_ctx.h
@@ -203,6 +203,7 @@
   int vif_strip_mask = 0x2;
   int vif_strip_seg = 0;
   int adm_mode = pqa::ADM_AUTO;
+  bool adm_cone = true;
   int motion_mode = pqa::MOTION_AUTO;
   bool trace = false;
   bool prof = false;
diff --git a/pqa2_amd/csrc/pqa_debug.hip b/pqa2_amd/csrc/pqa_debug.hip
--- a/pqa2_amd/csrc/pqa_debug.hip
+++ b/pqa2_amd/csrc/pqa_debug.hip
@@ -1,3 +1,4 @@
+#include "adm_need.h"
 #include "pqa_ctx.h"
 
 using namespace pqa;
@@ -60,6 +61,17 @@
   const int strip_seg = ctx->vif_fixed ? -1 : (ctx->vif_strip_mask >> scale & 1) ? ctx->vif_strip_seg : -1;
   vif_strip_shape((int)scale, L.w, L.h, (int)n_frames, strip_seg, shape);
   for (int i = 0; i < 4; ++i) out4[i] = shape[i];
+  return PQA_OK;
+}
+
+int pqa_debug_adm_need(uint32_t width, uint32_t height, int32_t* out20) {
+  if (!out20 || width == 0 || height == 0 || width > 65536 || height > 65536) return PQA_EINVAL;
+  const AdmNeed n = adm_need((int)width, (int)height);
+  for (int s = 0; s < 4; ++s) {
+    out20[4 * s + 0] = n.rows[s].lo; out20[4 * s + 1] = n.rows[s].hi;
+    out20[4 * s + 2] = n.cols[s].lo; out20[4 * s + 3] = n.cols[s].hi;
+  }
+  out20[16] = n.in_rows.lo; out20[17] = n.in_rows.hi; out20[18] = n.in_cols.lo; out20[19] = n.in_cols.hi;
   return PQA_OK;
 }
 
```

Measured after the change: 23080 frames/s (median of 6 runs). +3.0%, better.
